# zxhuang1698/ZeroShape

Measured on AMD Instinct MI355X. Metric: sdf_query_points_per_sec_vox128, higher is better.
Workload: dtype f16x3

## Files before the change

### include/zeroshape_hip.h

```cpp
#ifndef ZEROSHAPE_HIP_H
#define ZEROSHAPE_HIP_H

#include <stddef.h>
#include <stdint.h>

#ifdef __cplusplus
extern "C" {
#endif

#define ZS_ABI_VERSION 41

int zs_abi_version(void);

const char *zs_last_error(void);


int zs_chamfer_forward(const float *xyz1, const float *xyz2, int b, int n, int m,
                       float *dist1, float *dist2, int *idx1, int *idx2, void *stream);

size_t zs_chamfer_workspace_bytes(int b, int n, int m);
int zs_chamfer_forward_ws(const float *xyz1, const float *xyz2, int b, int n, int m,
                          float *dist1, float *dist2, int *idx1, int *idx2,
                          void *workspace, size_t workspace_bytes, void *stream);

int zs_chamfer_backward(const float *xyz1, const float *xyz2, int b, int n, int m,
                        float *gradxyz1, float *gradxyz2,
                        const float *graddist1, const float *graddist2,
                        const int *idx1, const int *idx2, void *stream);


size_t zs_sdf_program_bytes(void);
size_t zs_sdf_prologue_scratch_bytes(void);
size_t zs_sdf_workspace_bytes(void);
size_t zs_sdf_attn_scratch_bytes(int batch, int m);

int zs_sdf_prologue(void *programs, size_t program_stride_bytes, const float *lat_params,
                    const float *latent_depth, int batch, void *scratch, void *stream);
#define ZS_SDF_POS_PERLAYER 1
int zs_sdf_prologue_ex(void *programs, size_t program_stride_bytes, const float *lat_params,
                       const float *latent_depth, int batch, void *scratch, int flags, void *stream);

int zs_sdf_verdict_stats(const float *got, const float *want, int batch, int m, float flip_band, float tol, float tol_occ,
                         float *stats, int *flags, void *stream);

int zs_sdf_query_points(const void *programs, size_t program_stride_bytes, int batch,
                        const float *points, int m, float *logits, float *attn,
                        const int *tile_mask, void *workspace, void *stream);

int zs_sdf_query_grid(const void *programs, size_t program_stride_bytes, int batch,
                      const float *axis, int G, int slice_begin, int slice_end,
                      int apply_sigmoid, float *out, const int *tile_mask, void *workspace,
                      void *stream);

size_t zs_sdf_grid_attn_zmean_scratch_bytes(int batch, int n_cols, int G, size_t cap_bytes);
int zs_sdf_grid_attn_zmean_chunk(int batch, int n_cols, int G, size_t cap_bytes, int *imgs_per_chunk ,
                                 int *cols_per_chunk );
int zs_sdf_grid_attn_zmean(const void *programs, size_t program_stride_bytes, int batch,
                           const float *axis, int G, const int *columns, int n_cols, float *zmean,
                           void *workspace, void *scratch, size_t scratch_bytes, void *stream);

int zs_attn_frames(const float *zmean, int batch, int n_cols, const int *frame_col, int n_frames,
                   const float *images, int H, int W, const uint8_t *lut, int R, float *frames, void *stream);

int zs_sdf_split_programs(const void *programs, size_t program_stride_bytes, void *split_programs,
                          size_t split_stride_bytes, int batch, void *stream);
int zs_sdf_query_points_split(const void *split_programs, size_t program_stride_bytes, int batch,
                              const float *points, int m, float *logits, int *tile_flags,
                              void *workspace, void *stream);
int zs_sdf_query_grid_split(const void *split_programs, size_t program_stride_bytes, int batch,
                            const float *axis, int G, int slice_begin, int slice_end,
                            int apply_sigmoid, float *out, int *tile_flags, void *workspace,
                            void *stream);

int zs_sdf_block0_tables(const void *split_programs, size_t program_stride_bytes, int batch, float *tables, void *stream);

int zs_sdf_query_grid_range(const void *programs, size_t program_stride_bytes, int batch,
                            const float *axis, int G, long long point_begin, long long point_end,
                            int apply_sigmoid, float *out, const int *tile_mask, void *workspace,
                            void *stream);
int zs_sdf_query_grid_range_split(const void *split_programs, size_t program_stride_bytes, int batch,
                                  const float *axis, int G, long long point_begin,
                                  long long point_end, int apply_sigmoid, float *out,
                                  int *tile_flags, void *workspace, void *stream);

size_t zs_bf_grid_bytes(void);
size_t zs_bf_scratch_bytes(void);
int zs_bf_lower_bounds(const float *pred, int n, const float *gt_normalized, int m,
                       const float *rotations, int k, float *grid_gt, float *grid_pred,
                       void *scratch, float *lower_bounds, void *stream);

int zs_pose_max_batch(void);
size_t zs_pose_scratch_bytes(int n, int m, int count);
size_t zs_pose_best_bytes(void);
int zs_pose_best_init(float *best, void *stream);
int zs_pose_search_batch(const float *pred, int n, const float *gt_normalized, int m,
                         const float *rotations, const int *order, int count, int index_offset,
                         const float *lower_bound, const float *thresholds6, float *best,
                         void *scratch, void *stream);
size_t zs_pose_grid_bytes(int n, int m, int count);
int zs_pose_gt_grid(const float *gt_normalized, int m, void *grids, void *stream);
int zs_pose_search_batch_grid(const float *pred, int n, const float *gt_normalized, int m, const float *rotations,
                              const int *order, int count, int index_offset, const float *lower_bound,
                              const float *thresholds6, float *best, void *scratch, void *grids, const float *pred_stats,
                              void *stream);
size_t zs_morton_scratch_bytes(int n);
int zs_morton_sort(const float *points, int n, float *sorted, int *perm, float *tile_boxes, int tile, void *scratch,
                   void *stream);
size_t zs_str_scratch_bytes(int n);
int zs_str_sort(const float *points, int n, float *sorted, int *perm, void *scratch, void *stream);
size_t zs_pose_pack_bytes(int points);
int zs_pose_pack(const float *sorted_points, int points, float *pack, void *stream);
size_t zs_pose_sorted_scratch_bytes(int n, int m, int count);
int zs_pose_search_batch_sorted(const float *pred, const float *pred_sorted, int n, const float *gt_sorted,
                                const float *gt_pack, int m, const float *rotations, const int *order, int count,
                                int index_offset, const float *lower_bound, const float *thresholds6, float *best,
                                void *scratch, int mode, void *stream);
int zs_pose_apply(const float *pred, int n, const float *rotations, const int *index, float *out,
                  void *scratch, void *stream);
int zs_normalize_pc(const float *pc, int b, int n, float *out, void *scratch, void *stream);
int zs_standardize_pc(const float *pc, int b, int n, float *out, void *stream);
size_t zs_icp_scratch_bytes(int b);
int zs_icp_step(const float *x1, int n, const float *x2, int m, const int *idx1, int b, float *x1_out, void *scratch,
                void *stream);
int zs_fscore(const float *dist1, int n, const float *dist2, int m, int b, const float *thresholds,
              int n_thresholds, float *out, void *stream);

size_t zs_mc_scratch_bytes(int G);
size_t zs_mesh_sample_scratch_doubles(int n_tris);
int zs_mc_count(const float *vol, int G, float iso, const uint8_t *tri_count, void *scratch,
                int *total, void *stream);
int zs_mc_emit(const float *vol, int G, float iso, const int8_t *tri_table, int table_stride,
               const uint8_t *tri_count, const void *scratch, float scale, float offset,
               float *tris, int n_tris, void *stream);
int zs_mesh_sample(const float *tris, int n_tris, int n_samples, uint64_t seed, double *cum_area,
                   float *points, void *stream);


size_t zs_mesh_stats_scratch_bytes(int n_tris);
int zs_mesh_stats(const float *tris, int n_tris, float *out, void *scratch, void *stream);

size_t zs_render_zbuffer_bytes(int frames, int H, int W);
int zs_render_frames(const float *tris, int n_tris, const float *xform, const float *cams,
                     int frames, int H, int W, float yfov, float znear, const float *base_rgb,
                     uint8_t *rgb, float *depth, int *tri, void *zbuffer, void *stream);

int zs_intr_param2mtx(const float *params, int batch, int H, int W, float *intr, void *stream);
int zs_unproj_depth(const float *depth, const float *intr, int batch, int H, int W, float *points,
                    void *stream);
int zs_valid_norm_fac(const float *points, const uint8_t *mask, int batch, int n, float *mean,
                      float *max_dist, void *stream);
int zs_masked_resample(const float *map, const float *mask, int batch, int channels, int H, int W,
                       int Ho, int Wo, float bg, float *out, float *mask_out, void *stream);
int zs_seen_surface(const float *depth, const float *intr, const float *mask, int batch, int H, int W,
                    int Ho, int Wo, float *seen_points, float *mean, float *scale, float *coord_dsp,
                    float *mask_dsp, void *stream);
size_t zs_seen_surface_workspace_bytes(int batch);
int zs_seen_surface_ws(const float *depth, const float *intr, const float *mask, int batch, int H, int W,
                       int Ho, int Wo, float *seen_points, float *mean, float *scale, float *coord_dsp,
                       float *mask_dsp, void *workspace, void *stream);

#define ZS_DEPTH_PRED_IS_DISPARITY 1
#define ZS_DEPTH_SOLVE_ONLY 2
int zs_depth_metrics(const float *prediction, const float *target, const float *mask, int batch, int n,
                     int flags, float depth_cap, const float *thresholds,
                     int n_thresholds, float *metrics, float *prediction_depth, float *scale_shift,
                     void *stream);

#define ZS_ACT_NONE 0
#define ZS_ACT_RELU 1
#define ZS_ACT_GELU 2
#define ZS_ACT_RELU_CLAMP1 3
#define ZS_ACT_SOFTPLUS 4
#define ZS_CONV_IN_RELU 1
#define ZS_CONV_FORCE_LARGE 2
#define ZS_CONV_FORCE_SMALL 4
#define ZS_CONV_F16X3 16
#define ZS_CONV_SPLIT_SMALL 32
#define ZS_CONV_STREAM_K 64
#define ZS_CONV_STREAM_K_ALWAYS 256
#define ZS_CONV_W_PRESPLIT 128
#define ZS_CONV_IN_DILATE2 8
#define ZS_CONV_FORCE_TILE256 1024
#define ZS_CONV_OUT_K16 2048
#define ZS_CONV_IN_K16 4096
#define ZS_CONV_IN_UPSAMPLE2 512
size_t zs_conv2d_packed_floats(int Cin, int Cout, int kh, int kw);
int zs_conv2d_presplit_weight(const float *packed_w, float *split_w, int Cin, int Cout, int kh, int kw, void *stream);
int zs_conv2d_presplit_weight_multi(const void *const *packed, void *const *split, const int *cout_pad,
                                    const unsigned long long *pair_prefix, int n, unsigned long long total_pairs,
                                    void *stream);
int zs_conv2d_nhwc(const float *in, const float *packed_w, const float *scale, const float *shift,
                   const float *res1, const float *res2, float *out, int batch, int Hin, int Win, int Cin,
                   int Hout, int Wout, int Cout, int kh, int kw, int stride, int pad_t, int pad_l, int flags,
                   float in_scale, float in_shift, int act, void *stream);
size_t zs_conv2d_splitk_workspace_bytes(void);
int zs_conv2d_nhwc_ws(const float *in, const float *packed_w, const float *scale, const float *shift,
                   const float *res1, const float *res2, float *out, int batch, int Hin, int Win, int Cin,
                   int Hout, int Wout, int Cout, int kh, int kw, int stride, int pad_t, int pad_l, int flags,
                   float in_scale, float in_shift, int act, void *workspace, void *stream);

typedef struct zs_conv_fuse {
    int in_mode, in_tiles, in_groups;
    int in_gshift;
    const float *in_stats, *in_gamma, *in_beta;
    float in_eps;
    int out_mode, out_groups;
    float *out_stats;
} zs_conv_fuse;
int zs_conv2d_nhwc_fused(const float *in, const float *packed_w, const float *scale, const float *shift,
                         const float *res1, const float *res2, float *out, int batch, int Hin, int Win,
                         int Cin, int Hout, int Wout, int Cout, int kh, int kw, int stride, int pad_t,
                         int pad_l, int flags, float in_scale, float in_shift, int act, const zs_conv_fuse *fuse,
                         void *workspace, void *stream);
int zs_conv2d_fused_cols(int M, int Cout);
int zs_conv2d_k16_ok(int M, int Cin, int Cout, int flags, int ln_in_tiles, int row_stats_out, int has_res);
int zs_gn_relu_max_pool_nhwc(const float *x, const float *stats, int tiles, const float *gamma, const float *beta,
                             float *table, float *y, int batch, int Hin, int Win, int C, int Hout, int Wout, int k,
                             int stride, int pad_t, int pad_l, float eps, void *stream);
int zs_group_norm_apply_stats(const float *x, const float *stats, int tiles, const float *gamma, const float *beta,
                              const float *residual, const float *res_stats, int res_tiles, const float *res_gamma,
                              const float *res_beta, float *y, int batch, int HW, int C, float eps, int relu, void *stream);
int zs_conv3x3_tail_nhwc(const float *in, const float *packed_w, const float *scale, const float *shift, float *out,
                         int batch, int H, int W, int Cin, int Cout, int flags, int act, const float *tail_w,
                         const float *tail_b, int tail_act, void *stream);
int zs_group_norm_nhwc(const float *x, const float *gamma, const float *beta, const float *residual, float *y,
                       int batch, int HW, int C, int groups, float eps, int relu, void *stream);
size_t zs_group_norm_workspace_bytes(int batch, int HW, int C, int groups);
int zs_group_norm_nhwc_ws(const float *x, const float *gamma, const float *beta, const float *residual, float *y,
                          int batch, int HW, int C, int groups, float eps, int relu, void *workspace, void *stream);
int zs_layer_norm(const float *x, const float *gamma, const float *beta, float *y, int rows, int C, float eps,
                  void *stream);
int zs_attention(const float *qkv, float *out, int batch, int L, int heads, int head_dim, void *stream);
int zs_attention_split(const float *qkv, float *out, int batch, int L, int heads, int head_dim, void *stream);
int zs_max_pool_nhwc(const float *x, float *y, int batch, int Hin, int Win, int C, int Hout, int Wout, int k,
                     int stride, int pad_t, int pad_l, void *stream);
int zs_global_mean_nhwc(const float *x, float *y, int batch, int HW, int C, void *stream);
int zs_upsample2x_nhwc(const float *x, float *y, int batch, int Hin, int Win, int C, void *stream);
int zs_nchw_to_nhwc(const float *x, const float *mask, float *y, int batch, int C, int HW, int Cpad,
                    void *stream);
int zs_nhwc_to_nchw(const float *x, float *y, int batch, int C, int HW, void *stream);
int zs_assemble_tokens(const float *feat, const float *cls, const float *pos, float *tokens, int batch, int n,
                       int C, void *stream);
int zs_readout_concat(const float *tokens, float *out, int batch, int n, int C, void *stream);
int zs_window_tokens(const float *emb, const uint8_t *mask, const float *invalid_token, const float *cls,
                     const float *pos, float *out, int batch, int H, int W, int C, int win, void *stream);

typedef struct zs_tensor_entry {
    float *param;
    const float *grad;
    float *exp_avg, *exp_avg_sq;
    unsigned long long n;
    float lr, weight_decay;
} zs_tensor_entry;

int zs_pack_conv_weight(const float *w, float *packed, int Cout, int Cin, int cin0, int CinTot, int kh, int kw,
                        int dgrad, void *stream);
typedef struct zs_pack_entry {
    const float *src;
    float *dst;
    int Cout, Cin, cin0, ld, taps, dgrad, K16, NPad;
} zs_pack_entry;
int zs_pack_chunk_elems(void);
int zs_pack_entry_chunks(int Cout, int Cin, int taps, int dgrad, int K16, int NPad);
int zs_pack_conv_weight_multi(const zs_pack_entry *table, const int *chunk_entry, const unsigned long long *chunk_start,
                              int n_chunks, void *stream);
int zs_pack_entry_inline_split(int Cout, int Cin, int taps, int dgrad);
int zs_pack_conv_weight_multi_split(const zs_pack_entry *table, const int *chunk_entry,
                                    const unsigned long long *chunk_start, int n_chunks, float *const *split_dst,
                                    int split_only, void *stream);
size_t zs_conv2d_wgrad_workspace_bytes(int batch, int Hout, int Wout, int Cin, int Cout, int kh, int kw);
int zs_conv2d_wgrad(const float *in, const float *dy, float *dw, float *db, void *workspace, int batch, int Hin, int Win,
                    int CinP, int Hout, int Wout, int Cout, int kh, int kw, int stride, int pad_t, int pad_l,
                    int flags, float in_scale, float in_shift, int Cin, int cin0, int CinTot, int accumulate,
                    void *stream);
int zs_conv2d_dgrad_small_cin(const float *dy, const float *w, float *dx, int batch, int H, int W, int CinP, int Hout,
                              int Wout, int Cout, int kh, int kw, int stride, int pad_t, int pad_l, int Cin, int cin0,
                              int CinTot, float scale, void *stream);
int zs_standardize_weight(const float *w, float *out, int Cout, int n, float eps, void *stream);
typedef struct zs_std_entry {
    const float *w;
    float *out;
    int rows, n;
    float eps;
    int pad;
} zs_std_entry;
int zs_standardize_weight_multi(const zs_std_entry *table, const int *row_prefix, int n_entries, int total_rows, void *stream);
int zs_standardize_weight_bwd(const float *w, const float *grad_out, float *dw, int Cout, int n, float eps,
                              void *stream);
int zs_act_forward(const float *x, float *y, size_t n, int act, float beta, void *stream);
int zs_act_backward(const float *dy, const float *ref, float *dx, size_t n, int act, float beta, void *stream);
int zs_posenc3d(const float *points, size_t n, int L, float *out, int stride, void *stream);
int zs_add_scaled_rows(const float *x, const float *branch, const float *scale, float *y, int batch,
                       size_t per_sample, void *stream);
size_t zs_column_sum_workspace_bytes(int rows, int C);
int zs_column_sum(const float *x, float *out, int rows, int C, float scale, void *workspace, void *stream);
size_t zs_layer_norm_bwd_workspace_bytes(int rows, int C);
int zs_layer_norm_bwd(const float *dy, const float *x, const float *gamma, float *dx, float *dgamma, float *dbeta,
                      int rows, int C, float eps, void *workspace, void *stream);
int zs_layer_norm_bwd_add(const float *dy, const float *x, const float *gamma, const float *add, float *dx, float *dgamma,
                          float *dbeta, int rows, int C, float eps, void *workspace, void *stream);
size_t zs_attention_bwd_workspace_bytes(int batch, int L, int heads);
int zs_attention_bwd(const float *qkv, const float *dout, float *dqkv, void *workspace, int batch, int L, int heads,
                     int head_dim, void *stream);
int zs_point_attention(const float *qkv_points, const float *qkv_latent, float *out, int batch, int M, int Ll,
                       int heads, int head_dim, void *stream);
int zs_point_attention_probs(const float *qkv_points, const float *qkv_latent, float *attn, int batch, int M, int Ll,
                             int heads, int head_dim, float weight, int accumulate, void *stream);
size_t zs_point_attention_bwd_workspace_bytes(int batch, int M, int Ll, int heads);
int zs_point_attention_bwd(const float *qkv_points, const float *qkv_latent, const float *dout, float *dqkv_points,
                           float *dqkv_latent, int accumulate_latent, void *workspace, int batch, int M, int Ll,
                           int heads, int head_dim, void *stream);
size_t zs_bce_logits_workspace_bytes(size_t n);
int zs_bce_logits(const float *logits, const float *sdf, size_t n, float impt_thres, float impt_weight, float *loss,
                  void *workspace, void *stream);
int zs_bce_logits_bwd(const float *logits, const float *sdf, size_t n, float impt_thres, float impt_weight,
                      const float *grad_loss, float *dlogits, void *stream);
int zs_erode_mask(const float *mask, int batch, int H, int W, int pool, float *out, void *stream);
size_t zs_midas_loss_workspace_bytes(int batch);
int zs_midas_loss(const float *prediction, const float *target, const float *mask, int batch, int H, int W, float alpha,
                  int scales, int inverse_depth, float *loss, void *workspace, void *stream);
int zs_midas_loss_bwd(const float *prediction, const float *target, const float *mask, int batch, int H, int W,
                      float alpha, int scales, int inverse_depth, const void *workspace, const float *grad_loss,
                      float *dprediction, void *stream);
int zs_intr_loss(const float *seen_pred, const float *seen_gt, const float *mask, size_t n, float *out2, void *stream);
int zs_intr_loss_bwd(const float *seen_pred, const float *seen_gt, const float *mask, size_t n, const float *out2,
                     const float *grad_loss, float *dseen_pred, void *stream);
int zs_multi_tensor_chunk_elems(void);
int zs_adamw_multi(const zs_tensor_entry *table, const int *chunk_tensor, const unsigned long long *chunk_start,
                   int n_chunks, float beta1, float beta2, float eps, int step, const float *grad_scale,
                   const int *skipped_steps, void *stream);
int zs_copy_multi(const zs_tensor_entry *table, const int *chunk_tensor, const unsigned long long *chunk_start,
                  int n_chunks, float scale, void *stream);
int zs_sumsq_multi(const zs_tensor_entry *table, const int *chunk_tensor, const unsigned long long *chunk_start,
                   int n_chunks, float *partial, float *sumsq, void *stream);

size_t zs_batch_norm_workspace_bytes(int rows, int C);
int zs_batch_norm_train(const float *x, const float *gamma, const float *beta, const float *residual, float *y,
                        float *running_mean, float *running_var, float *save_mean, float *save_rstd, int rows, int C,
                        float eps, float momentum, int relu, void *workspace, void *stream);
int zs_batch_norm_bwd(const float *x, const float *dy, const float *y_relu, const float *gamma, const float *save_mean,
                      const float *save_rstd, float *dx, float *dresidual, float *dgamma, float *dbeta, int rows, int C,
                      void *workspace, void *stream);
size_t zs_group_norm_bwd_workspace_bytes(int batch, int C);
int zs_group_norm_bwd(const float *x, const float *dy, const float *y_relu, const float *gamma, float *dx,
                      float *dresidual, float *dgamma, float *dbeta, int batch, int HW, int C, int groups, float eps,
                      void *workspace, void *stream);
int zs_max_pool_bwd_nhwc(const float *x, const float *dy, float *dx, int batch, int Hin, int Win, int C, int Hout,
                         int Wout, int k, int stride, int pad_t, int pad_l, void *stream);
int zs_global_mean_bwd_nhwc(const float *dy, float *dx, int batch, int HW, int C, void *stream);
int zs_upsample2x_bwd_nhwc(const float *dy, float *dx, int batch, int Hin, int Win, int C, void *stream);
int zs_nhwc_to_nchw_masked(const float *x, const float *mask, float *y, int batch, int C, int HW, int Cpad,
                           void *stream);
int zs_seen_surface_bwd(const float *depth, const float *intr, const float *mask, const float *mean, const float *scale,
                        const float *d_seen_points, const float *d_coord_dsp, int batch, int H, int W, float *d_depth,
                        float *d_intr, void *stream);
int zs_intr_param2mtx_bwd(const float *params, const float *d_intr, int batch, int H, int W, float *d_params,
                          void *stream);
int zs_window_tokens_bwd(const float *d_out, const uint8_t *mask, float *d_emb, float *d_inv_rows, float *d_cls_rows,
                         int batch, int H, int W, int C, int win, void *stream);
int zs_coord_dsp2_bwd(const float *d_dsp, const float *mask, const float *mask_dsp, float *d_full, int batch, int H,
                      int W, void *stream);
int zs_transform_points(const float *points, const float *pose, const float *mean, const float *scale, float *out,
                        int batch, int n, void *stream);
int zs_resize_bilinear_nhwc(const float *x, float *y, int Hi, int Wi, int Ho, int Wo, int C, int backward,
                            void *stream);
int zs_readout_concat_bwd(const float *dout, float *dtokens, int batch, int n, int C, void *stream);

#ifdef __cplusplus
}
#endif
#endif
```

### zeroshape_amd/_lib.py

```python
import contextlib
import ctypes
import os

_HERE = os.path.dirname(os.path.abspath(__file__))
LIB_PATH = os.environ.get("ZS_LIB_PATH") or os.path.join(_HERE, "libzeroshape_hip.so")

_c_void_p = ctypes.c_void_p
_c_int = ctypes.c_int
_c_size_t = ctypes.c_size_t
_c_float = ctypes.c_float

class ConvFuse(ctypes.Structure):
    _fields_ = [("in_mode", ctypes.c_int), ("in_tiles", ctypes.c_int), ("in_groups", ctypes.c_int), ("in_gshift", ctypes.c_int),
                ("in_stats", ctypes.c_void_p), ("in_gamma", ctypes.c_void_p), ("in_beta", ctypes.c_void_p),
                ("in_eps", ctypes.c_float), ("out_mode", ctypes.c_int), ("out_groups", ctypes.c_int),
                ("out_stats", ctypes.c_void_p)]


SIGNATURES = {
    "zs_abi_version": (_c_int, []),
    "zs_last_error": (ctypes.c_char_p, []),
    "zs_chamfer_forward": (_c_int, [_c_void_p, _c_void_p, _c_int, _c_int, _c_int,
                                    _c_void_p, _c_void_p, _c_void_p, _c_void_p, _c_void_p]),
    "zs_chamfer_workspace_bytes": (_c_size_t, [_c_int, _c_int, _c_int]),
    "zs_chamfer_forward_ws": (_c_int, [_c_void_p, _c_void_p, _c_int, _c_int, _c_int,
                                       _c_void_p, _c_void_p, _c_void_p, _c_void_p, _c_void_p, _c_size_t,
                                       _c_void_p]),
    "zs_chamfer_backward": (_c_int, [_c_void_p, _c_void_p, _c_int, _c_int, _c_int,
                                     _c_void_p, _c_void_p, _c_void_p, _c_void_p,
                                     _c_void_p, _c_void_p, _c_void_p]),
    "zs_sdf_program_bytes": (_c_size_t, []),
    "zs_sdf_prologue_scratch_bytes": (_c_size_t, []),
    "zs_sdf_workspace_bytes": (_c_size_t, []),
    "zs_sdf_attn_scratch_bytes": (_c_size_t, [_c_int, _c_int]),
    "zs_sdf_prologue": (_c_int, [_c_void_p, _c_size_t, _c_void_p, _c_void_p, _c_int,
                                 _c_void_p, _c_void_p]),
    "zs_sdf_prologue_ex": (_c_int, [_c_void_p, _c_size_t, _c_void_p, _c_void_p, _c_int,
                                    _c_void_p, _c_int, _c_void_p]),
    "zs_sdf_verdict_stats": (_c_int, [_c_void_p, _c_void_p, _c_int, _c_int, _c_float, _c_float, _c_float, _c_void_p, _c_void_p,
                                      _c_void_p]),
    "zs_sdf_query_points": (_c_int, [_c_void_p, _c_size_t, _c_int, _c_void_p, _c_int,
                                     _c_void_p, _c_void_p, _c_void_p, _c_void_p, _c_void_p]),
    "zs_sdf_query_grid": (_c_int, [_c_void_p, _c_size_t, _c_int, _c_void_p, _c_int, _c_int,
                                   _c_int, _c_int, _c_void_p, _c_void_p, _c_void_p, _c_void_p]),
    "zs_sdf_grid_attn_zmean_scratch_bytes": (_c_size_t, [_c_int, _c_int, _c_int, _c_size_t]),
    "zs_sdf_grid_attn_zmean_chunk": (_c_int, [_c_int, _c_int, _c_int, _c_size_t, ctypes.POINTER(_c_int),
                                              ctypes.POINTER(_c_int)]),
    "zs_sdf_grid_attn_zmean": (_c_int, [_c_void_p, _c_size_t, _c_int, _c_void_p, _c_int, _c_void_p, _c_int, _c_void_p,
                                        _c_void_p, _c_void_p, _c_size_t, _c_void_p]),
    "zs_attn_frames": (_c_int, [_c_void_p, _c_int, _c_int, _c_void_p, _c_int, _c_void_p, _c_int, _c_int, _c_void_p, _c_int,
                                _c_void_p, _c_void_p]),
    "zs_sdf_split_programs": (_c_int, [_c_void_p, _c_size_t, _c_void_p, _c_size_t, _c_int, _c_void_p]),
    "zs_sdf_block0_tables": (_c_int, [_c_void_p, _c_size_t, _c_int, _c_void_p, _c_void_p]),
    "zs_sdf_query_points_split": (_c_int, [_c_void_p, _c_size_t, _c_int, _c_void_p, _c_int,
                                           _c_void_p, _c_void_p, _c_void_p, _c_void_p]),
    "zs_sdf_query_grid_split": (_c_int, [_c_void_p, _c_size_t, _c_int, _c_void_p, _c_int, _c_int,
                                         _c_int, _c_int, _c_void_p, _c_void_p, _c_void_p, _c_void_p]),
    "zs_sdf_query_grid_range": (_c_int, [_c_void_p, _c_size_t, _c_int, _c_void_p, _c_int, ctypes.c_longlong,
                                         ctypes.c_longlong, _c_int, _c_void_p, _c_void_p, _c_void_p, _c_void_p]),
    "zs_sdf_query_grid_range_split": (_c_int, [_c_void_p, _c_size_t, _c_int, _c_void_p, _c_int,
                                               ctypes.c_longlong, ctypes.c_longlong, _c_int, _c_void_p,
                                               _c_void_p, _c_void_p, _c_void_p]),
    "zs_erode_mask": (_c_int, [_c_void_p, _c_int, _c_int, _c_int, _c_int, _c_void_p, _c_void_p]),
    "zs_bf_grid_bytes": (_c_size_t, []),
    "zs_bf_scratch_bytes": (_c_size_t, []),
    "zs_bf_lower_bounds": (_c_int, [_c_void_p, _c_int, _c_void_p, _c_int, _c_void_p, _c_int, _c_void_p,
                                    _c_void_p, _c_void_p, _c_void_p, _c_void_p]),
    "zs_pose_max_batch": (_c_int, []),
    "zs_pose_scratch_bytes": (_c_size_t, [_c_int, _c_int, _c_int]),
    "zs_pose_best_bytes": (_c_size_t, []),
    "zs_pose_best_init": (_c_int, [_c_void_p, _c_void_p]),
    "zs_pose_search_batch": (_c_int, [_c_void_p, _c_int, _c_void_p, _c_int, _c_void_p, _c_void_p, _c_int, _c_int,
                                      _c_void_p, _c_void_p, _c_void_p, _c_void_p, _c_void_p]),
    "zs_pose_grid_bytes": (_c_size_t, [_c_int, _c_int, _c_int]),
    "zs_pose_gt_grid": (_c_int, [_c_void_p, _c_int, _c_void_p, _c_void_p]),
    "zs_pose_search_batch_grid": (_c_int, [_c_void_p, _c_int, _c_void_p, _c_int, _c_void_p, _c_void_p, _c_int, _c_int,
                                           _c_void_p, _c_void_p, _c_void_p, _c_void_p, _c_void_p, _c_void_p, _c_void_p]),
    "zs_morton_scratch_bytes": (_c_size_t, [_c_int]),
    "zs_morton_sort": (_c_int, [_c_void_p, _c_int, _c_void_p, _c_void_p, _c_void_p, _c_int, _c_void_p, _c_void_p]),
    "zs_str_scratch_bytes": (_c_size_t, [_c_int]),
    "zs_str_sort": (_c_int, [_c_void_p, _c_int, _c_void_p, _c_void_p, _c_void_p, _c_void_p]),
    "zs_pose_pack_bytes": (_c_size_t, [_c_int]),
    "zs_pose_pack": (_c_int, [_c_void_p, _c_int, _c_void_p, _c_void_p]),
    "zs_pose_sorted_scratch_bytes": (_c_size_t, [_c_int, _c_int, _c_int]),
    "zs_pose_search_batch_sorted": (_c_int, [_c_void_p, _c_void_p, _c_int, _c_void_p, _c_void_p, _c_int, _c_void_p,
                                             _c_void_p, _c_int, _c_int, _c_void_p, _c_void_p, _c_void_p, _c_void_p,
                                             _c_int, _c_void_p]),
    "zs_pose_apply": (_c_int, [_c_void_p, _c_int, _c_void_p, _c_void_p, _c_void_p, _c_void_p, _c_void_p]),
    "zs_standardize_pc": (_c_int, [_c_void_p, _c_int, _c_int, _c_void_p, _c_void_p]),
    "zs_icp_scratch_bytes": (_c_size_t, [_c_int]),
    "zs_icp_step": (_c_int, [_c_void_p, _c_int, _c_void_p, _c_int, _c_void_p, _c_int, _c_void_p, _c_void_p, _c_void_p]),
    "zs_normalize_pc": (_c_int, [_c_void_p, _c_int, _c_int, _c_void_p, _c_void_p, _c_void_p]),
    "zs_fscore": (_c_int, [_c_void_p, _c_int, _c_void_p, _c_int, _c_int, _c_void_p, _c_int, _c_void_p, _c_void_p]),
    "zs_mc_scratch_bytes": (_c_size_t, [_c_int]),
    "zs_mesh_sample_scratch_doubles": (_c_size_t, [_c_int]),
    "zs_mc_count": (_c_int, [_c_void_p, _c_int, ctypes.c_float, _c_void_p, _c_void_p, _c_void_p, _c_void_p]),
    "zs_mc_emit": (_c_int, [_c_void_p, _c_int, ctypes.c_float, _c_void_p, _c_int, _c_void_p, _c_void_p,
                            ctypes.c_float, ctypes.c_float, _c_void_p, _c_int, _c_void_p]),
    "zs_mesh_sample": (_c_int, [_c_void_p, _c_int, _c_int, ctypes.c_uint64, _c_void_p, _c_void_p, _c_void_p]),
    "zs_mesh_stats_scratch_bytes": (_c_size_t, [_c_int]),
    "zs_mesh_stats": (_c_int, [_c_void_p, _c_int, _c_void_p, _c_void_p, _c_void_p]),
    "zs_render_zbuffer_bytes": (_c_size_t, [_c_int, _c_int, _c_int]),
    "zs_render_frames": (_c_int, [_c_void_p, _c_int, ctypes.POINTER(_c_float), _c_void_p, _c_int, _c_int, _c_int, _c_float,
                                  _c_float, ctypes.POINTER(_c_float), _c_void_p, _c_void_p, _c_void_p, _c_void_p, _c_void_p]),
    "zs_intr_param2mtx": (_c_int, [_c_void_p, _c_int, _c_int, _c_int, _c_void_p, _c_void_p]),
    "zs_unproj_depth": (_c_int, [_c_void_p, _c_void_p, _c_int, _c_int, _c_int, _c_void_p, _c_void_p]),
    "zs_valid_norm_fac": (_c_int, [_c_void_p, _c_void_p, _c_int, _c_int, _c_void_p, _c_void_p, _c_void_p]),
    "zs_masked_resample": (_c_int, [_c_void_p, _c_void_p, _c_int, _c_int, _c_int, _c_int, _c_int, _c_int,
                                    ctypes.c_float, _c_void_p, _c_void_p, _c_void_p]),
    "zs_seen_surface": (_c_int, [_c_void_p, _c_void_p, _c_void_p, _c_int, _c_int, _c_int, _c_int, _c_int,
                                 _c_void_p, _c_void_p, _c_void_p, _c_void_p, _c_void_p, _c_void_p]),
    "zs_seen_surface_workspace_bytes": (_c_size_t, [_c_int]),
    "zs_seen_surface_ws": (_c_int, [_c_void_p, _c_void_p, _c_void_p, _c_int, _c_int, _c_int, _c_int, _c_int,
                                    _c_void_p, _c_void_p, _c_void_p, _c_void_p, _c_void_p, _c_void_p, _c_void_p]),
    "zs_depth_metrics": (_c_int, [_c_void_p, _c_void_p, _c_void_p, _c_int, _c_int, _c_int, ctypes.c_float,
                                  ctypes.POINTER(ctypes.c_float), _c_int, _c_void_p, _c_void_p, _c_void_p,
                                  _c_void_p]),
    "zs_conv2d_packed_floats": (_c_size_t, [_c_int, _c_int, _c_int, _c_int]),
    "zs_conv2d_presplit_weight": (_c_int, [_c_void_p, _c_void_p, _c_int, _c_int, _c_int, _c_int, _c_void_p]),
    "zs_conv2d_nhwc": (_c_int, [_c_void_p] * 7 + [_c_int] * 13 + [ctypes.c_float, ctypes.c_float, _c_int,
                                                                  _c_void_p]),
    "zs_conv2d_splitk_workspace_bytes": (_c_size_t, []),
    "zs_conv2d_presplit_weight_multi": (_c_int, [_c_void_p] * 4 + [_c_int, ctypes.c_ulonglong, _c_void_p]),
    "zs_conv3x3_tail_nhwc": (_c_int, [_c_void_p] * 5 + [_c_int] * 7 + [_c_void_p, _c_void_p, _c_int, _c_void_p]),
    "zs_conv2d_nhwc_ws": (_c_int, [_c_void_p] * 7 + [_c_int] * 13 + [ctypes.c_float, ctypes.c_float, _c_int,
                                                                     _c_void_p, _c_void_p]),
    "zs_conv2d_nhwc_fused": (_c_int, [_c_void_p] * 7 + [_c_int] * 13 + [ctypes.c_float, ctypes.c_float, _c_int,
                                                                        _c_void_p, _c_void_p, _c_void_p]),
    "zs_conv2d_fused_cols": (_c_int, [_c_int, _c_int]),
    "zs_conv2d_k16_ok": (_c_int, [_c_int] * 7),
    "zs_gn_relu_max_pool_nhwc": (_c_int, [_c_void_p, _c_void_p, _c_int] + [_c_void_p] * 4 + [_c_int] * 10 + [ctypes.c_float, _c_void_p]),
    "zs_group_norm_apply_stats": (_c_int, [_c_void_p, _c_void_p, _c_int] + [_c_void_p] * 4 + [_c_int] + [_c_void_p] * 3 +
                                  [_c_int, _c_int, _c_int, ctypes.c_float, _c_int, _c_void_p]),
    "zs_group_norm_nhwc": (_c_int, [_c_void_p] * 5 + [_c_int, _c_int, _c_int, _c_int, ctypes.c_float, _c_int,
                                                      _c_void_p]),
    "zs_group_norm_workspace_bytes": (_c_size_t, [_c_int, _c_int, _c_int, _c_int]),
    "zs_group_norm_nhwc_ws": (_c_int, [_c_void_p] * 5 + [_c_int, _c_int, _c_int, _c_int, ctypes.c_float, _c_int,
                                       _c_void_p, _c_void_p]),
    "zs_layer_norm": (_c_int, [_c_void_p] * 4 + [_c_int, _c_int, ctypes.c_float, _c_void_p]),
    "zs_attention": (_c_int, [_c_void_p, _c_void_p, _c_int, _c_int, _c_int, _c_int, _c_void_p]),
    "zs_attention_split": (_c_int, [_c_void_p, _c_void_p, _c_int, _c_int, _c_int, _c_int, _c_void_p]),
    "zs_max_pool_nhwc": (_c_int, [_c_void_p, _c_void_p] + [_c_int] * 10 + [_c_void_p]),
    "zs_global_mean_nhwc": (_c_int, [_c_void_p, _c_void_p, _c_int, _c_int, _c_int, _c_void_p]),
    "zs_upsample2x_nhwc": (_c_int, [_c_void_p, _c_void_p, _c_int, _c_int, _c_int, _c_int, _c_void_p]),
    "zs_nchw_to_nhwc": (_c_int, [_c_void_p, _c_void_p, _c_void_p, _c_int, _c_int, _c_int, _c_int, _c_void_p]),
    "zs_window_tokens": (_c_int, [_c_void_p] * 6 + [_c_int] * 5 + [_c_void_p]),
    "zs_nhwc_to_nchw": (_c_int, [_c_void_p, _c_void_p, _c_int, _c_int, _c_int, _c_void_p]),
    "zs_assemble_tokens": (_c_int, [_c_void_p] * 4 + [_c_int, _c_int, _c_int, _c_void_p]),
    "zs_readout_concat": (_c_int, [_c_void_p, _c_void_p, _c_int, _c_int, _c_int, _c_void_p]),
    "zs_pack_conv_weight": (_c_int, [_c_void_p, _c_void_p] + [_c_int] * 7 + [_c_void_p]),
    "zs_pack_chunk_elems": (_c_int, []),
    "zs_pack_entry_chunks": (_c_int, [_c_int] * 6),
    "zs_pack_conv_weight_multi": (_c_int, [_c_void_p, _c_void_p, _c_void_p, _c_int, _c_void_p]),
    "zs_pack_entry_inline_split": (_c_int, [_c_int] * 4),
    "zs_pack_conv_weight_multi_split": (_c_int, [_c_void_p, _c_void_p, _c_void_p, _c_int, _c_void_p, _c_int, _c_void_p]),
    "zs_conv2d_wgrad_workspace_bytes": (_c_size_t, [_c_int] * 7),
    "zs_conv2d_wgrad": (_c_int, [_c_void_p] * 5 + [_c_int] * 13 + [_c_float, _c_float] + [_c_int] * 4 + [_c_void_p]),
    "zs_conv2d_dgrad_small_cin": (_c_int, [_c_void_p] * 3 + [_c_int] * 15 + [_c_float, _c_void_p]),
    "zs_standardize_weight": (_c_int, [_c_void_p, _c_void_p, _c_int, _c_int, _c_float, _c_void_p]),
    "zs_standardize_weight_multi": (_c_int, [_c_void_p, _c_void_p, _c_int, _c_int, _c_void_p]),
    "zs_standardize_weight_bwd": (_c_int, [_c_void_p, _c_void_p, _c_void_p, _c_int, _c_int, _c_float, _c_void_p]),
    "zs_act_forward": (_c_int, [_c_void_p, _c_void_p, _c_size_t, _c_int, _c_float, _c_void_p]),
    "zs_act_backward": (_c_int, [_c_void_p, _c_void_p, _c_void_p, _c_size_t, _c_int, _c_float, _c_void_p]),
    "zs_posenc3d": (_c_int, [_c_void_p, _c_size_t, _c_int, _c_void_p, _c_int, _c_void_p]),
    "zs_add_scaled_rows": (_c_int, [_c_void_p] * 4 + [_c_int, _c_size_t, _c_void_p]),
    "zs_column_sum_workspace_bytes": (_c_size_t, [_c_int, _c_int]),
    "zs_column_sum": (_c_int, [_c_void_p, _c_void_p, _c_int, _c_int, _c_float, _c_void_p, _c_void_p]),
    "zs_layer_norm_bwd_workspace_bytes": (_c_size_t, [_c_int, _c_int]),
    "zs_layer_norm_bwd": (_c_int, [_c_void_p] * 6 + [_c_int, _c_int, _c_float, _c_void_p, _c_void_p]),
    "zs_layer_norm_bwd_add": (_c_int, [_c_void_p] * 7 + [_c_int, _c_int, _c_float, _c_void_p, _c_void_p]),
    "zs_attention_bwd_workspace_bytes": (_c_size_t, [_c_int, _c_int, _c_int]),
    "zs_attention_bwd": (_c_int, [_c_void_p] * 4 + [_c_int] * 4 + [_c_void_p]),
    "zs_point_attention": (_c_int, [_c_void_p] * 3 + [_c_int] * 5 + [_c_void_p]),
    "zs_point_attention_probs": (_c_int, [_c_void_p, _c_void_p, _c_void_p, _c_int, _c_int, _c_int, _c_int, _c_int, _c_float, _c_int,
                                          _c_void_p]),
    "zs_point_attention_bwd_workspace_bytes": (_c_size_t, [_c_int] * 4),
    "zs_point_attention_bwd": (_c_int, [_c_void_p] * 5 + [_c_int, _c_void_p] + [_c_int] * 5 + [_c_void_p]),
    "zs_bce_logits_workspace_bytes": (_c_size_t, [_c_size_t]),
    "zs_bce_logits": (_c_int, [_c_void_p, _c_void_p, _c_size_t, _c_float, _c_float, _c_void_p, _c_void_p,
                               _c_void_p]),
    "zs_bce_logits_bwd": (_c_int, [_c_void_p, _c_void_p, _c_size_t, _c_float, _c_float, _c_void_p, _c_void_p,
                                   _c_void_p]),
    "zs_midas_loss_workspace_bytes": (_c_size_t, [_c_int]),
    "zs_midas_loss": (_c_int, [_c_void_p] * 3 + [_c_int] * 3 + [_c_float, _c_int, _c_int, _c_void_p, _c_void_p, _c_void_p]),
    "zs_midas_loss_bwd": (_c_int, [_c_void_p] * 3 + [_c_int] * 3 + [_c_float, _c_int, _c_int, _c_void_p, _c_void_p,
                                                                    _c_void_p, _c_void_p]),
    "zs_intr_loss": (_c_int, [_c_void_p] * 3 + [_c_size_t, _c_void_p, _c_void_p]),
    "zs_intr_loss_bwd": (_c_int, [_c_void_p] * 3 + [_c_size_t] + [_c_void_p] * 4),
    "zs_multi_tensor_chunk_elems": (_c_int, []),
    "zs_adamw_multi": (_c_int, [_c_void_p, _c_void_p, _c_void_p, _c_int, _c_float, _c_float, _c_float, _c_int,
                                _c_void_p, _c_void_p, _c_void_p]),
    "zs_copy_multi": (_c_int, [_c_void_p, _c_void_p, _c_void_p, _c_int, _c_float, _c_void_p]),
    "zs_sumsq_multi": (_c_int, [_c_void_p, _c_void_p, _c_void_p, _c_int, _c_void_p, _c_void_p, _c_void_p]),
    "zs_batch_norm_workspace_bytes": (_c_size_t, [_c_int, _c_int]),
    "zs_batch_norm_train": (_c_int, [_c_void_p] * 9 + [_c_int, _c_int, _c_float, _c_float, _c_int, _c_void_p,
                                                       _c_void_p]),
    "zs_batch_norm_bwd": (_c_int, [_c_void_p] * 10 + [_c_int, _c_int, _c_void_p, _c_void_p]),
    "zs_group_norm_bwd_workspace_bytes": (_c_size_t, [_c_int, _c_int]),
    "zs_group_norm_bwd": (_c_int, [_c_void_p] * 8 + [_c_int, _c_int, _c_int, _c_int, _c_float, _c_void_p, _c_void_p]),
    "zs_max_pool_bwd_nhwc": (_c_int, [_c_void_p] * 3 + [_c_int] * 10 + [_c_void_p]),
    "zs_global_mean_bwd_nhwc": (_c_int, [_c_void_p, _c_void_p, _c_int, _c_int, _c_int, _c_void_p]),
    "zs_upsample2x_bwd_nhwc": (_c_int, [_c_void_p, _c_void_p, _c_int, _c_int, _c_int, _c_int, _c_void_p]),
    "zs_nhwc_to_nchw_masked": (_c_int, [_c_void_p, _c_void_p, _c_void_p, _c_int, _c_int, _c_int, _c_int, _c_void_p]),
    "zs_seen_surface_bwd": (_c_int, [_c_void_p] * 7 + [_c_int, _c_int, _c_int, _c_void_p, _c_void_p, _c_void_p]),
    "zs_intr_param2mtx_bwd": (_c_int, [_c_void_p, _c_void_p, _c_int, _c_int, _c_int, _c_void_p, _c_void_p]),
    "zs_window_tokens_bwd": (_c_int, [_c_void_p] * 5 + [_c_int] * 5 + [_c_void_p]),
    "zs_coord_dsp2_bwd": (_c_int, [_c_void_p] * 4 + [_c_int] * 3 + [_c_void_p]),
    "zs_transform_points": (_c_int, [_c_void_p] * 5 + [_c_int, _c_int, _c_void_p]),
    "zs_resize_bilinear_nhwc": (_c_int, [_c_void_p, _c_void_p] + [_c_int] * 6 + [_c_void_p]),
    "zs_readout_concat_bwd": (_c_int, [_c_void_p, _c_void_p, _c_int, _c_int, _c_int, _c_void_p]),
}

ABI_VERSION = 41
_lib = None


class ZeroShapeHipError(RuntimeError):
    pass


def load():
    global _lib
    if _lib is not None:
        return _lib
    if not os.path.exists(LIB_PATH):
        raise ZeroShapeHipError(
            "HIP library not built: %s is missing (run `python -m zeroshape_amd.build`). "
            "zeroshape_amd has no CPU/PyTorch fallback for this path." % LIB_PATH)
    import torch
    try:
        lib = ctypes.CDLL(LIB_PATH)
    except OSError as e:
        raise ZeroShapeHipError("cannot load %s: %s" % (LIB_PATH, e)) from e
    for name, (res, args) in SIGNATURES.items():
        try:
            fn = getattr(lib, name)
        except AttributeError as e:
            raise ZeroShapeHipError("%s does not export %s" % (LIB_PATH, name)) from e
        fn.restype = res
        fn.argtypes = args
    v = lib.zs_abi_version()
    if v != ABI_VERSION:
        raise ZeroShapeHipError("ABI mismatch: library %d, binding %d" % (v, ABI_VERSION))
    _lib = lib
    return lib


CALLS = [0]


def check(rc, what):
    CALLS[0] += 1
    if rc != 1:
        msg = load().zs_last_error()
        raise ZeroShapeHipError("%s failed: %s" % (what, (msg or b"").decode(errors="replace")))


def ptr(t):
    return None if t is None else ctypes.c_void_p(t.data_ptr())


def current_stream_ptr(device=None):
    import torch
    idx = getattr(device, "index", device)
    if idx is None:
        idx = torch.cuda.current_device()
    return ctypes.c_void_p(torch._C._cuda_getCurrentRawStream(idx))


_NULL_GUARD = contextlib.nullcontext()


def on(device):
    import torch
    idx = getattr(device, "index", device)
    if idx is None or idx == torch.cuda.current_device():
        return _NULL_GUARD
    return torch.cuda.device(device)
```

### zeroshape_amd/csrc/sdf_decoder_split.hip

```cpp
#include "zs_common.h"
#include <stdlib.h>
#include "sdf_layout.h"
#include "sdf_math.h"
#include "zs_split16.h"
#include "../../include/zeroshape_hip.h"

#include <math.h>
#include <stdint.h>
#include <type_traits>

namespace {

using namespace zs::lay;
using zs::dm::gelu_erf;
using zs::dm::softplus100;

typedef float f32x16 __attribute__((ext_vector_type(16)));
typedef float f32x4 __attribute__((ext_vector_type(4)));
typedef float f32x2 __attribute__((ext_vector_type(2)));
typedef unsigned u32x4 __attribute__((ext_vector_type(4)));

constexpr float S_GUARD = 64.0f;
constexpr int WAVES = 4;
constexpr int PTS_PER_WAVE = 32;
constexpr int PTS_PER_BLOCK = WAVES * PTS_PER_WAVE;
constexpr int MAX_WGS = 256;
constexpr int KB_U4 = 128;
constexpr int CK = 8;
constexpr int KPW = CK / WAVES;
constexpr int CHUNK_BYTES = CK * KB_U4 * 16;
constexpr int NBUF = 2;
constexpr int KB_TOTAL = G_TOTAL / 2;
constexpr int PRM_WINDOW = 4096;
constexpr int STAGE_FLOATS = NBUF * CHUNK_BYTES / 4;
constexpr int SLAB_TILES = NT - 1;
constexpr int SLAB_U4 = SLAB_TILES * 4 * 64;
constexpr int ZTILES_F4 = NT * 4 * 64;
constexpr int ZSLAB_F4 = 3 * ZTILES_F4;
constexpr int LDS_FLOATS = PRM_WINDOW + STAGE_FLOATS + WAVES * SLAB_U4 * 4;
static_assert(LDS_FLOATS * 4 == 160 * 1024, "the kernel owns the whole LDS of a CU");
static_assert(KB_TOTAL % CK == 0 && CK % WAVES == 0 && KPW * 2048 <= 4096, "chunking");
static_assert((RING * GROUP_FLOATS + PARAM_FLOATS) * 4 >= NBUF * CHUNK_BYTES, "prefetch stays inside the program");

constexpr int W_PP = P_PP;
constexpr int W_BLK = P_BLK0;
constexpr int W_IA = P_LNFG;
constexpr int W_IB = P_IMPL_PAIR + P_IMPL_PAIR_STRIDE;
static_assert(P_BLK_STRIDE <= PRM_WINDOW && W_IB - W_IA <= PRM_WINDOW && P_USED - W_IB <= PRM_WINDOW,
              "params windows");

#define DEV __device__ __forceinline__
#ifdef ZS_FENCE_SCHED
#define ZS_FENCE __builtin_amdgcn_sched_barrier(0)
#else
#define ZS_FENCE do { } while (0)
#endif

DEV void pin(u32x4 &a, u32x4 &b) { asm volatile("" : "+v"(a), "+v"(b) : : "memory"); }

using zs::s16::mfma3;
using zs::s16::split2;

struct PT {
    u32x4 v[4];
};
template <typename T>
DEV PT pack_tile(const T &x) {
    PT p;
#pragma unroll
    for (int j = 0; j < 2; j++)
#pragma unroll
        for (int i = 0; i < 4; i++) {
            unsigned h, l;
            split2(x[8 * j + 2 * i], x[8 * j + 2 * i + 1], h, l);
            p.v[2 * j][i] = h;
            p.v[2 * j + 1][i] = l;
        }
    return p;
}

DEV void glds_kblocks(const char *gsrc, unsigned lds_dst) {
#ifdef ZS_EXP_NO_DMA
    if (gsrc != nullptr) return;
#endif
#ifndef ZS_DMA_MOD
#define ZS_DMA_MOD ""
#endif
    asm volatile("s_mov_b32 m0, %1\n\ts_nop 0\n\tglobal_load_lds_dwordx4 %0, off" ZS_DMA_MOD
                 "\n\tglobal_load_lds_dwordx4 %0, off offset:1024" ZS_DMA_MOD
                 "\n\tglobal_load_lds_dwordx4 %0, off offset:2048" ZS_DMA_MOD
                 "\n\tglobal_load_lds_dwordx4 %0, off offset:3072" ZS_DMA_MOD
                 :
                 : "v"(gsrc), "s"(lds_dst)
                 : "memory");
}

struct AStream {
    const u32x4 *buf[NBUF];
    unsigned dst[NBUF];
    u32x4 hi, lo;
    const char *gsrc;

    DEV void init(const char *prog, u32x4 *stage, unsigned stage_addr, int wave, int lane, int first_byte = 0) {
        const char *g = prog + first_byte + wave * (KPW * KB_U4 * 16) + lane * 16;
        asm volatile("s_waitcnt vmcnt(0) lgkmcnt(0)\n\ts_barrier" ::: "memory");
#pragma unroll
        for (int i = 0; i < NBUF; i++) {
            buf[i] = stage + i * (CK * KB_U4) + lane;
            dst[i] = stage_addr + i * CHUNK_BYTES + wave * (KPW * KB_U4 * 16);
            glds_kblocks(g + i * CHUNK_BYTES, dst[i]);
        }
        gsrc = g + NBUF * CHUNK_BYTES;
        asm volatile("s_waitcnt vmcnt(4)\n\ts_barrier" ::: "memory");
        hi = buf[0][0];
        lo = buf[0][64];
    }
    template <int EXTRA_VM = 0>
    DEV void step(int pos, u32x4 &ahi, u32x4 &alo) {
        ahi = hi;
        alo = lo;
        if (pos == CK - 1) {
            static_assert(EXTRA_VM == 0 || EXTRA_VM == 4, "wait-count variants");
            if (EXTRA_VM == 4)
                asm volatile("s_waitcnt vmcnt(4) lgkmcnt(0)\n\ts_barrier" ::: "memory");
            else
                asm volatile("s_waitcnt vmcnt(0) lgkmcnt(0)\n\ts_barrier" ::: "memory");
            glds_kblocks(gsrc, dst[0]);
            gsrc += CHUNK_BYTES;
            const u32x4 *t = buf[0];
            const unsigned u = dst[0];
            buf[0] = buf[1];
            dst[0] = dst[1];
            buf[1] = t;
            dst[1] = u;
            hi = buf[0][0];
            lo = buf[0][64];
        } else {
#ifndef ZS_EXP_NO_AREAD
            hi = buf[0][(pos + 1) * KB_U4];
            lo = buf[0][(pos + 1) * KB_U4 + 64];
#endif
        }
    }
    DEV void skip(int bytes) { gsrc += bytes; }
    DEV void drain() { asm volatile("s_waitcnt vmcnt(0) lgkmcnt(0)" ::: "memory"); }
};

struct Slab {
    u32x4 *fl;
    PT t7;
    DEV void store(int tile, const PT &p) {
        if (tile == SLAB_TILES) {
            t7 = p;
        } else {
#pragma unroll
            for (int q = 0; q < 4; q++) fl[(tile * 4 + q) * 64] = p.v[q];
        }
    }
};

DEV f32x16 zero16() {
    f32x16 v;
#pragma unroll
    for (int r = 0; r < 16; r++) v[r] = 0.f;
    return v;
}

struct NoSide {
    DEV void operator()(int, int) const {}
};
template <typename SIDE>
DEV void mfma3_gaps(f32x16 &acc, const u32x4 &ahi, const u32x4 &alo, const u32x4 &bhi, const u32x4 &blo, int kb,
                    SIDE &side) {
    using zs::s16::as_h;
    if (std::is_same<SIDE, NoSide>::value) {
        mfma3(acc, ahi, alo, bhi, blo);
        return;
    }
    acc = __builtin_amdgcn_mfma_f32_32x32x16_f16(as_h(alo), as_h(bhi), acc, 0, 0, 0);
    ZS_FENCE;
    side(kb, 0);
    ZS_FENCE;
    acc = __builtin_amdgcn_mfma_f32_32x32x16_f16(as_h(ahi), as_h(blo), acc, 0, 0, 0);
    ZS_FENCE;
    side(kb, 1);
    ZS_FENCE;
    acc = __builtin_amdgcn_mfma_f32_32x32x16_f16(as_h(ahi), as_h(bhi), acc, 0, 0, 0);
    ZS_FENCE;
    side(kb, 2);
    ZS_FENCE;
}

struct TilePacker {
    PT p;
    float prev;
    DEV void feed(int kb, float v) {
        if (kb & 1) {
            unsigned h, l;
            split2(prev, v, h, l);
            p.v[2 * (kb >> 3)][(kb & 7) >> 1] = h;
            p.v[2 * (kb >> 3) + 1][(kb & 7) >> 1] = l;
        }
        prev = v;
    }
};

struct GeluStager {
    float x, u, q, t, e, p;
    DEV void s0(float v) {
        x = v;
        u = fabsf(v) * 0.70710678118654752440f;
        q = (u * u) * -1.44269504088896340736f;
    }
    DEV void s1() { t = __builtin_amdgcn_rcpf(fmaf(0.3275911f, u, 1.0f)); }
    DEV void s2() {
        e = __builtin_amdgcn_exp2f(q);
        p = fmaf(0.75052702f, t, -1.02753365f);
    }
    DEV void s3() {
        p = fmaf(p, t, 1.00509130f);
        p = fmaf(p, t, -0.20116957f);
        p = fmaf(p, t, 0.18019173f);
        p = p * t;
        u = u * p;
    }
    DEV float s4() const { return fmaf(-u, e, fmaxf(x, 0.0f)); }
    DEV float all(float v) {
        s0(v); s1(); s2(); s3();
        return s4();
    }
    DEV void stage(int st, float v, int idx, TilePacker &pk) {
        if (st == 0) s0(v);
        else if (st == 1) s1();
        else if (st == 2) s2();
        else if (st == 3) s3();
        else if (st == 4) pk.feed(idx, s4());
    }
};
struct SoftplusStager {
    float x, t;
    DEV void s0(float v) {
        x = v;
        t = __builtin_amdgcn_exp2f(fabsf(v) * -144.26950408889634074f);
    }
    DEV void s1() { t = __builtin_amdgcn_logf(1.0f + t); }
    DEV float s2() const { return fmaf(t, 0.0069314718055994530942f, fmaxf(x, 0.0f)); }
};

DEV float kblock_gelu(f32x16 &acc, const u32x4 &ahi, const u32x4 &alo, const u32x4 &bhi, const u32x4 &blo, float x) {
    float u, q, d, t, e, m, p;
    const float c0 = 0.70710678118654752440f, c1 = 0.3275911f, c2 = -1.02753365f;
    asm volatile(
#ifndef ZS_EXP_TWO_TERM
                 "v_mfma_f32_32x32x16_f16 %[acc], %[alo], %[bh], %[acc]\n\t"
#endif
                 "v_mul_f32_e64 %[u], |%[x]|, %[c0]\n\t"
                 "v_mul_f32_e32 %[q], %[u], %[u]\n\t"
                 "v_mul_f32_e32 %[q], 0xbfb8aa3b, %[q]\n\t"
                 "v_fma_f32 %[d], %[u], %[c1], 1.0\n\t"
                 "v_mfma_f32_32x32x16_f16 %[acc], %[ahi], %[bl], %[acc]\n\t"
                 "v_rcp_f32_e32 %[t], %[d]\n\t"
                 "v_exp_f32_e32 %[e], %[q]\n\t"
                 "v_max_f32_e32 %[m], 0, %[x]\n\t"
                 "v_mfma_f32_32x32x16_f16 %[acc], %[ahi], %[bh], %[acc]\n\t"
                 "v_fmamk_f32 %[p], %[t], 0x3f40228a, %[c2]\n\t"
                 "v_fmaak_f32 %[p], %[p], %[t], 0x3f80a6d5\n\t"
                 "v_fmaak_f32 %[p], %[p], %[t], 0xbe4dff65\n\t"
                 "v_fmaak_f32 %[p], %[p], %[t], 0x3e38842e\n\t"
                 "v_mul_f32_e64 %[p], %[t], -%[p]\n\t"
                 "v_mul_f32_e32 %[p], %[u], %[p]\n\t"
                 "v_fmac_f32_e32 %[m], %[p], %[e]"
                 : [acc] "+v"(acc), [u] "=&v"(u), [q] "=&v"(q), [d] "=&v"(d), [t] "=&v"(t), [e] "=&v"(e), [m] "=&v"(m),
                   [p] "=&v"(p)
                 : [alo] "v"(alo), [ahi] "v"(ahi), [bh] "v"(bhi), [bl] "v"(blo), [x] "v"(x), [c0] "s"(c0), [c1] "s"(c1),
                   [c2] "v"(c2));
    return m;
}
DEV float kblock_softplus(f32x16 &acc, const u32x4 &ahi, const u32x4 &alo, const u32x4 &bhi, const u32x4 &blo, float x) {
    float t, m;
    const float c0 = -144.26950408889634074f;
    asm volatile(
#ifndef ZS_EXP_TWO_TERM
                 "v_mfma_f32_32x32x16_f16 %[acc], %[alo], %[bh], %[acc]\n\t"
#endif
                 "v_mul_f32_e64 %[t], |%[x]|, %[c0]\n\t"
                 "v_exp_f32_e32 %[t], %[t]\n\t"
                 "v_mfma_f32_32x32x16_f16 %[acc], %[ahi], %[bl], %[acc]\n\t"
                 "v_max_f32_e32 %[m], 0, %[x]\n\t"
                 "v_add_f32_e32 %[t], 1.0, %[t]\n\t"
                 "v_log_f32_e32 %[t], %[t]\n\t"
                 "v_mfma_f32_32x32x16_f16 %[acc], %[ahi], %[bh], %[acc]\n\t"
                 "s_nop 0\n\t"
                 "v_fmac_f32_e32 %[m], 0x3be32166, %[t]"
                 : [acc] "+v"(acc), [t] "=&v"(t), [m] "=&v"(m)
                 : [alo] "v"(alo), [ahi] "v"(ahi), [bh] "v"(bhi), [bl] "v"(blo), [x] "v"(x), [c0] "s"(c0));
    return m;
}

DEV void mfma_settle(f32x16 &acc) { asm volatile("s_nop 7\n\ts_nop 3" : "+v"(acc)); }

template <int KT, int EXTRA_VM = 0, typename SIDE = NoSide>
DEV void gemm_reg(AStream &s, const PT *X, f32x16 &acc, SIDE side = SIDE()) {
#pragma unroll
    for (int kt = 0; kt < KT; kt++)
#pragma unroll
        for (int j = 0; j < 2; j++) {
            u32x4 ahi, alo;
            s.step((kt * 2 + j) & (CK - 1), ahi, alo);
            pin(ahi, alo);
            mfma3_gaps(acc, ahi, alo, X[kt].v[2 * j], X[kt].v[2 * j + 1], kt * 2 + j, side);
        }
}
template <typename SIDE>
DEV void mfma3_breg(f32x16 &acc, const u32x4 &ahi, const u32x4 &alo, const u32x4 &bhi, const u32x4 &blo, int kb,
                    SIDE &side) {
    asm volatile("s_nop 1\n\tv_mfma_f32_32x32x16_f16 %0, %1, %2, %0" : "+v"(acc) : "v"(alo), "a"(bhi));
    ZS_FENCE;
    side(kb, 0);
    ZS_FENCE;
    asm volatile("s_nop 1\n\tv_mfma_f32_32x32x16_f16 %0, %1, %2, %0" : "+v"(acc) : "v"(ahi), "a"(blo));
    ZS_FENCE;
    side(kb, 1);
    ZS_FENCE;
    asm volatile("s_nop 1\n\tv_mfma_f32_32x32x16_f16 %0, %1, %2, %0" : "+v"(acc) : "v"(ahi), "a"(bhi));
    ZS_FENCE;
    side(kb, 2);
    ZS_FENCE;
}
template <int KT, typename SIDE = NoSide>
DEV void gemm_areg(AStream &s, const PT *X, f32x16 &acc, SIDE side = SIDE()) {
#pragma unroll
    for (int kt = 0; kt < KT; kt++)
#pragma unroll
        for (int j = 0; j < 2; j++) {
            u32x4 ahi, alo;
            s.step((kt * 2 + j) & (CK - 1), ahi, alo);
            pin(ahi, alo);
            mfma3_breg(acc, ahi, alo, X[kt].v[2 * j], X[kt].v[2 * j + 1], kt * 2 + j, side);
        }
}
template <typename SIDE>
DEV void mfma3_cacc(f32x16 &acc, const u32x4 &ahi, const u32x4 &alo, const u32x4 &bhi, const u32x4 &blo, int kb,
                    SIDE &side) {
    asm volatile("s_nop 1\n\tv_mfma_f32_32x32x16_f16 %0, %1, %2, %0" : "+a"(acc) : "v"(alo), "v"(bhi));
    ZS_FENCE;
    side(kb, 0);
    ZS_FENCE;
    asm volatile("s_nop 1\n\tv_mfma_f32_32x32x16_f16 %0, %1, %2, %0" : "+a"(acc) : "v"(ahi), "v"(blo));
    ZS_FENCE;
    side(kb, 1);
    ZS_FENCE;
    asm volatile("s_nop 1\n\tv_mfma_f32_32x32x16_f16 %0, %1, %2, %0" : "+a"(acc) : "v"(ahi), "v"(bhi));
    ZS_FENCE;
    side(kb, 2);
    ZS_FENCE;
}
template <bool YACC = false, typename SIDE = NoSide>
DEV void gemm_one(AStream &s, const PT &X, f32x16 &acc, int pos0, int kb0 = 0, SIDE side = SIDE()) {
#pragma unroll
    for (int j = 0; j < 2; j++) {
        u32x4 ahi, alo;
        s.step((pos0 + j) & (CK - 1), ahi, alo);
        pin(ahi, alo);
        if (YACC)
            mfma3_cacc(acc, ahi, alo, X.v[2 * j], X.v[2 * j + 1], kb0 + j, side);
        else
            mfma3_gaps(acc, ahi, alo, X.v[2 * j], X.v[2 * j + 1], kb0 + j, side);
    }
}
DEV void slab_b(const Slab &sl, int kb, u32x4 &bh, u32x4 &bl) {
    if (kb >= SLAB_TILES * 2) {
        bh = sl.t7.v[(kb & 1) * 2];
        bl = sl.t7.v[(kb & 1) * 2 + 1];
    } else {
        bh = sl.fl[kb * KB_U4];
        bl = sl.fl[kb * KB_U4 + 64];
    }
}
template <typename SIDE = NoSide>
DEV void gemm_lds(AStream &s, const Slab &sl, f32x16 &acc, int pos0 = 0, SIDE side = SIDE()) {
    u32x4 bh, bl;
    slab_b(sl, 0, bh, bl);
#pragma unroll
    for (int kb = 0; kb < NT * 2; kb++) {
        u32x4 ahi, alo;
        s.step((pos0 + kb) & (CK - 1), ahi, alo);
        u32x4 nh = bh, nl = bl;
        if (kb + 1 < NT * 2) slab_b(sl, kb + 1, nh, nl);
        pin(ahi, alo);
        mfma3_gaps(acc, ahi, alo, bh, bl, kb, side);
        bh = nh;
        bl = nl;
    }
}

template <int ACT, typename FIN, typename TAIL>
DEV void gemm_lds_act(AStream &s, const Slab &sl, f32x16 &acc, const f32x16 &cur, FIN fin, TAIL tail) {
    u32x4 bh, bl;
    slab_b(sl, 0, bh, bl);
#pragma unroll
    for (int kb = 0; kb < NT * 2; kb++) {
        u32x4 ahi, alo;
        s.step(kb & (CK - 1), ahi, alo);
        u32x4 nh = bh, nl = bl;
        if (kb + 1 < NT * 2) slab_b(sl, kb + 1, nh, nl);
        const float r = ACT == 0 ? kblock_gelu(acc, ahi, alo, bh, bl, cur[kb]) : kblock_softplus(acc, ahi, alo, bh, bl, cur[kb]);
        bh = nh;
        bl = nl;
        fin(kb, r);
        tail(kb);
    }
}
template <int ACT, typename FIN, typename TAIL>
DEV void gemm_reg_act(AStream &s, const PT *X, f32x16 &acc, const f32x16 &cur, FIN fin, TAIL tail) {
#pragma unroll
    for (int kt = 0; kt < NT; kt++)
#pragma unroll
        for (int j = 0; j < 2; j++) {
            u32x4 ahi, alo;
            const int kb = kt * 2 + j;
            s.step(kb & (CK - 1), ahi, alo);
            const float r = ACT == 0 ? kblock_gelu(acc, ahi, alo, X[kt].v[2 * j], X[kt].v[2 * j + 1], cur[kb])
                                     : kblock_softplus(acc, ahi, alo, X[kt].v[2 * j], X[kt].v[2 * j + 1], cur[kb]);
            fin(kb, r);
            tail(kb);
        }
}

#ifndef ZS_SPLIT_PERMLANE
DEV float half_sum(float v) { return v + __shfl_xor(v, 32, 64); }
DEV float half_max(float v) { return fmaxf(v, __shfl_xor(v, 32, 64)); }
#else
DEV void half_pair(float v, float &lo, float &hi) {
    lo = v;
    hi = v;
    asm volatile("s_nop 4\n\tv_permlane32_swap_b32 %0, %1\n\ts_nop 4" : "+v"(lo), "+v"(hi));
}
DEV float half_sum(float v) {
    float lo, hi;
    half_pair(v, lo, hi);
    return lo + hi;
}
#ifdef ZS_SPLIT_PERMLANE_SUM_ONLY
DEV float half_max(float v) { return fmaxf(v, __shfl_xor(v, 32, 64)); }
#else
DEV float half_max(float v) {
    float lo, hi;
    half_pair(v, lo, hi);
    return fmaxf(lo, hi);
}
#endif
#endif

DEV void rp(const float *prm, int off, int tile, int hi, float *v) {
    const f32x4 *q = reinterpret_cast<const f32x4 *>(prm + off + tile * 32 + hi * 16);
#pragma unroll
    for (int i = 0; i < 4; i++) {
        const f32x4 a = q[i];
        v[4 * i + 0] = a.x; v[4 * i + 1] = a.y; v[4 * i + 2] = a.z; v[4 * i + 3] = a.w;
    }
}
DEV f32x16 rp16(const float *prm, int off, int tile, int hi) {
    float t[16];
    rp(prm, off, tile, hi, t);
    f32x16 v;
#pragma unroll
    for (int r = 0; r < 16; r++) v[r] = t[r];
    return v;
}
constexpr int B0_BPROJ = 0, B0_C = 256, B0_T = 1024;
static_assert(B0_T + HEADS * 3 * 128 == PRM_WINDOW, "the block-0 table is exactly one params window");
DEV f32x16 block0_qkv(const float *prm, int tile, int hi, float xr, float yr, float zr, float rstd) {
    f32x16 v = rp16(prm, B0_C, tile, hi);
    const f32x4 *q = reinterpret_cast<const f32x4 *>(prm + B0_T + tile * 128 + hi * 64);
#pragma unroll
    for (int r = 0; r < 16; r++) {
        const f32x4 w = q[r];
        v[r] = fmaf(w.z, zr, fmaf(w.y, yr, fmaf(w.x, xr, fmaf(w.w, rstd, v[r]))));
    }
    return v;
}
DEV f32x16 xyz_affine(const float *prm, int off, int tile, int hi, float x, float y, float z) {
    const f32x4 *q = reinterpret_cast<const f32x4 *>(prm + off + tile * 128 + hi * 64);
    f32x16 v;
#pragma unroll
    for (int r = 0; r < 16; r++) {
        const f32x4 w = q[r];
        v[r] = fmaf(w.z, z, fmaf(w.y, y, fmaf(w.x, x, w.w)));
    }
    return v;
}

struct XyzInit {
    const f32x4 *q;
    f32x4 w;
    f32x16 v;
    DEV void start(const float *prm, int off, int tile, int hi) {
        q = reinterpret_cast<const f32x4 *>(prm + off + tile * 128 + hi * 64);
        w = q[0];
    }
    DEV void step(int r, float x, float y, float z) {
        v[r] = fmaf(w.z, z, fmaf(w.y, y, fmaf(w.x, x, w.w)));
        if (r + 1 < 16) w = q[r + 1];
    }
};
struct RowInit {
    const f32x4 *q;
    f32x4 w;
    f32x16 v;
    DEV void start(const float *prm, int off, int tile, int hi) {
        q = reinterpret_cast<const f32x4 *>(prm + off + tile * 32 + hi * 16);
        w = q[0];
    }
    DEV void step(int r) {
        if ((r & 3) == 0) {
            v[r] = w.x; v[r + 1] = w.y; v[r + 2] = w.z; v[r + 3] = w.w;
            if (r + 4 < 16) w = q[(r >> 2) + 1];
        }
    }
};

DEV void ln_stats(const f32x16 *x, float &mean, float &rstd) {
    float s = 0.f;
#pragma unroll
    for (int kt = 0; kt < NT; kt++)
#pragma unroll
        for (int r = 0; r < 16; r++) s += x[kt][r];
    s = half_sum(s);
    mean = s * (1.0f / 256.0f);
    float v = 0.f;
#pragma unroll
    for (int kt = 0; kt < NT; kt++)
#pragma unroll
        for (int r = 0; r < 16; r++) {
            const float d = x[kt][r] - mean;
            v = fmaf(d, d, v);
        }
    v = half_sum(v);
    rstd = 1.0f / sqrtf(v * (1.0f / 256.0f) + 1e-6f);
}
DEV void layer_norm_lds(const f32x16 *x, Slab &sl, const float *prm, int g_off, int b_off, int hi) {
    float mean, rstd;
    ln_stats(x, mean, rstd);
#pragma unroll
    for (int kt = 0; kt < NT; kt++) {
        float g[16], b[16], t[16];
        rp(prm, g_off, kt, hi, g);
        rp(prm, b_off, kt, hi, b);
#pragma unroll
        for (int r = 0; r < 16; r++) t[r] = fmaf((x[kt][r] - mean) * rstd, g[r], b[r]);
        sl.store(kt, pack_tile(t));
    }
}

DEV void load_params(float *prm, const float *prog_params, int start, int count) {
    __syncthreads();
    const f32x4 *src = reinterpret_cast<const f32x4 *>(prog_params + start);
    f32x4 *dst = reinterpret_cast<f32x4 *>(prm);
    for (int i = threadIdx.x; i < count / 4; i += WAVES * 64) dst[i] = src[i];
    __syncthreads();
}

template <bool MASK>
DEV void attn_tile(AStream &s, const PT &q, f32x16 &o, float &m_run, float &z_run, float c, int hi,
                   int pos0) {
    f32x16 S = zero16();
    gemm_one(s, q, S, pos0);
    float mt = -INFINITY;
#pragma unroll
    for (int r = 0; r < 16; r++) {
        if (MASK) {
            const int rw = (r & 3) + 8 * (r >> 2) + 4 * hi;
            S[r] = rw < L - 32 * (LT - 1) ? S[r] : -INFINITY;
        }
        mt = fmaxf(mt, S[r]);
    }
    mt *= c;
    constexpr float LAZY = 8.0f;
    if (__builtin_amdgcn_ballot_w64(mt > m_run + LAZY) != 0) {
        mt = half_max(mt);
        const float m_new = fmaxf(m_run, mt);
        const float alpha = __builtin_amdgcn_exp2f(m_run - m_new);
        z_run *= alpha;
#pragma unroll
        for (int r = 0; r < 16; r++) o[r] *= alpha;
        m_run = m_new;
    }
    float zs_ = 0.f;
#pragma unroll
    for (int r = 0; r < 16; r++) {
        const float p = __builtin_amdgcn_exp2f(fmaf(S[r], c, -m_run));
        S[r] = p;
        zs_ += p;
    }
    z_run += zs_;
    gemm_one(s, pack_tile(S), o, pos0 + 2);
}

#ifdef ZS_EXP_TIMING
#define ZS_STAMP(i) do { if (dbg) dbg[i] = __builtin_amdgcn_s_memtime(); } while (0)
#else
#define ZS_STAMP(i) do { } while (0)
#endif
DEV float decode_tile(const char *prog, float *prm, u32x4 *stage, unsigned stage_addr, u32x4 *slab,
                      const float *tbl, float px, float py, float pz, int wave, int lane, float &guard,
                      unsigned long long *dbg) {
    const int hi = lane >> 5;
    const float *prog_params = reinterpret_cast<const float *>(prog) + REC_FLOATS;
    constexpr int QKV_BYTES = 3 * NT * 2 / CK * CHUNK_BYTES;
    static_assert(3 * NT * 2 % CK == 0, "AStream::skip passes whole chunks");
    AStream s;
    s.init(prog, stage, stage_addr, wave, lane, tbl ? QKV_BYTES : 0);
    Slab sl;
    sl.fl = slab;
    ZS_STAMP(0);

    load_params(prm, prog_params, W_PP, 1024);
    f32x16 y[NT];
#pragma unroll
    for (int kt = 0; kt < NT; kt++) y[kt] = xyz_affine(prm, 0, kt, hi, px, py, pz);

    ZS_STAMP(1);

    const float scale = 0.17677669529663688110f;

#pragma unroll 1
    for (int blk = 0; blk < BLOCKS; blk++) {
        const bool tab = blk == 0 && tbl != nullptr;
        float rstd0 = 0.f, xr = 0.f, yr = 0.f, zr = 0.f;
        if (tab) {
            load_params(prm, tbl, 0, PRM_WINDOW);
            float mean;
            ln_stats(y, mean, rstd0);
            xr = px * rstd0;
            yr = py * rstd0;
            zr = pz * rstd0;
        } else {
            load_params(prm, prog_params, W_BLK + blk * P_BLK_STRIDE, P_BLK_STRIDE);
            layer_norm_lds(y, sl, prm, PB_LN1G, PB_LN1B, hi);
        }
        ZS_STAMP(2 + blk * 4);
#pragma unroll
        for (int nt = 0; nt < NT; nt++) y[nt] += rp16(prm, tab ? B0_BPROJ : PB_BPROJ, nt, hi);

        auto head = [&](int hd, auto Ptag) {
            constexpr int P = decltype(Ptag)::value;
            f32x16 q, k, v;
            if (tab) {
                q = block0_qkv(prm, hd * 3 + 0, hi, xr, yr, zr, rstd0);
                k = block0_qkv(prm, hd * 3 + 1, hi, xr, yr, zr, rstd0);
                v = block0_qkv(prm, hd * 3 + 2, hi, xr, yr, zr, rstd0);
            } else {
                q = rp16(prm, PB_BQKV, hd * 3 + 0, hi);
                gemm_lds(s, sl, q, P);
                k = rp16(prm, PB_BQKV, hd * 3 + 1, hi);
                gemm_lds(s, sl, k, P);
                v = rp16(prm, PB_BQKV, hd * 3 + 2, hi);
                gemm_lds(s, sl, v, P);
            }

            const float c = scale * 1.44269504088896340736f;
            float s_self = 0.f;
            float qq = 0.f;
#pragma unroll
            for (int r = 0; r < 16; r++) {
                s_self = fmaf(q[r], k[r], s_self);
                qq = fmaf(q[r], q[r], qq);
            }
            s_self = half_sum(s_self) * c;
            {
                const float km = prog_params[P_KMAX + blk * HEADS + hd] * scale;
                guard = fmaxf(guard, half_sum(qq) * (km * km));
            }
            const PT qp = pack_tile(q);

            float m_run = -INFINITY, z_run = 0.f;
            f32x16 o = zero16();
#pragma unroll 1
            for (int l2 = 0; l2 < (LT - 1) / 2; l2++) {
                attn_tile<false>(s, qp, o, m_run, z_run, c, hi, P);
                attn_tile<false>(s, qp, o, m_run, z_run, c, hi, (P + 4) & (CK - 1));
            }
            attn_tile<true>(s, qp, o, m_run, z_run, c, hi, P);
            {
                const float m_new = fmaxf(m_run, s_self);
                const float alpha = __builtin_amdgcn_exp2f(m_run - m_new);
                const float p_self = __builtin_amdgcn_exp2f(s_self - m_new);
                const float z = fmaf(half_sum(z_run), alpha, p_self);
                const float inv = 1.0f / z;
                const float a_i = alpha * inv, p_i = p_self * inv;
#pragma unroll
                for (int r = 0; r < 16; r++) o[r] = fmaf(p_i, v[r], o[r] * a_i);
            }
            const PT op = pack_tile(o);
            const bool bump = tab && hd + 1 < HEADS;
            if (bump && (P == 4 || wave >= 2)) s.skip(QKV_BYTES);
#pragma unroll
            for (int nt = 0; nt < NT; nt++) {
                if (P == 0 && nt == 2 && bump && wave < 2) s.skip(QKV_BYTES);
                gemm_one(s, op, y[nt], (P + 4 + 2 * nt) & (CK - 1));
            }
        };
        static_assert((LT - 1) % 2 == 0 && (3 * NT * 2 + LT * 4 + NT * 2) % CK == 4, "head = 11.5 chunks");
#pragma unroll 1
        for (int hd = 0; hd < HEADS; hd += 2) {
            head(hd, std::integral_constant<int, 0>());
            head(hd + 1, std::integral_constant<int, 4>());
        }

        ZS_STAMP(3 + blk * 4);
        if (tab) load_params(prm, prog_params, W_BLK, P_BLK_STRIDE);
        layer_norm_lds(y, sl, prm, PB_LN2G, PB_LN2B, hi);
#pragma unroll
        for (int nt = 0; nt < NT; nt++) y[nt] += rp16(prm, PB_B2, nt, hi);
        ZS_STAMP(4 + blk * 4);
        RowInit bi;
        f32x16 hid = rp16(prm, PB_B1, 0, hi);
        bi.start(prm, PB_B1, 1, hi);
        gemm_lds(s, sl, hid, 0, [&](int kb, int g) {
            if (g == 2 && (kb & 3) == 1) bi.step(kb & ~3);
        });
#pragma unroll 1
        for (int ht = 0; ht < HT - 1; ht++) {
            f32x16 nxt = bi.v;
            bi.start(prm, PB_B1, ht + 2 < HT ? ht + 2 : HT - 1, hi);
            TilePacker e;
            gemm_lds_act<0>(s, sl, nxt, hid, [&](int kb, float r) { e.feed(kb, r); },
                            [&](int kb) { if ((kb & 3) == 1) bi.step(kb & ~3); });
#pragma unroll
            for (int nt = 0; nt < NT; nt++) gemm_one(s, e.p, y[nt], (2 * nt) & (CK - 1));
            hid = nxt;
        }
        {
#pragma unroll
            for (int r = 0; r < 16; r++) hid[r] = gelu_erf(hid[r]);
            const PT hp = pack_tile(hid);
#pragma unroll
            for (int nt = 0; nt < NT; nt++) gemm_one(s, hp, y[nt], (2 * nt) & (CK - 1));
        }
        ZS_STAMP(5 + blk * 4);
    }

    load_params(prm, prog_params, W_IA, W_IB - W_IA);
    float h[NT * 16];
    {
        float mean, rstd;
        ln_stats(y, mean, rstd);
#pragma unroll
        for (int kt = 0; kt < NT; kt++) {
            float g[16], b[16];
            rp(prm, P_LNFG - W_IA, kt, hi, g);
            rp(prm, P_LNFB - W_IA, kt, hi, b);
#pragma unroll
            for (int r = 0; r < 16; r++) h[kt * 16 + r] = fmaf((y[kt][r] - mean) * rstd, g[r], b[r]);
        }
    }
    ZS_STAMP(10);
    PT hp[NT];

#pragma unroll
    for (int kt = 0; kt < NT; kt++) hp[kt] = pack_tile(h + kt * 16);
    {
        f32x16 prev;
        XyzInit ini;
        ini.v = xyz_affine(prm, P_IMPL0 - W_IA, 0, hi, px, py, pz);
#pragma unroll
        for (int nt = 0; nt <= NT; nt++) {
            TilePacker e;
            if (nt < NT) {
                f32x16 acc = ini.v;
                if (nt + 1 < NT) ini.start(prm, P_IMPL0 - W_IA, nt + 1, hi);
                if (nt > 0)
                    gemm_reg_act<1>(s, hp, acc, prev, [&](int kb, float r) { e.feed(kb, r); },
                                    [&](int kb) { if (nt + 1 < NT) ini.step(kb, px, py, pz); });
                else
                    gemm_reg<NT, 0>(s, hp, acc, [&](int kb, int g) { if (g == 2) ini.step(kb, px, py, pz); });
                if (nt > 0) sl.store(nt - 1, e.p);
                prev = acc;
            } else {
                mfma_settle(prev);
#pragma unroll
                for (int kb = 0; kb < 16; kb++) e.feed(kb, softplus100(prev[kb]));
                sl.store(nt - 1, e.p);
            }
        }
    }
    ZS_STAMP(11);
    const float rsqrt2 = 0.70710678118654752440f;
    PT fp[NT];
#pragma unroll
    for (int kt = 0; kt < NT; kt++) {
        float t[16];
#pragma unroll
        for (int r = 0; r < 16; r++) t[r] = h[kt * 16 + r] * rsqrt2;
        fp[kt] = pack_tile(t);
    }
    const float sx = px * rsqrt2, sy = py * rsqrt2, sz = pz * rsqrt2;

    ZS_STAMP(12);
    {
        f32x16 prev;
        RowInit ini;
        ini.v = rp16(prm, P_IMPL1 - W_IA, 0, hi);
#pragma unroll
        for (int nt = 0; nt <= NT; nt++) {
            TilePacker e;
            if (nt < NT) {
                f32x16 acc = ini.v;
                if (nt + 1 < NT) ini.start(prm, P_IMPL1 - W_IA, nt + 1, hi);
                if (nt > 0)
                    gemm_lds_act<1>(s, sl, acc, prev, [&](int kb, float r) { e.feed(kb, r * rsqrt2); },
                                    [&](int kb) { if (nt + 1 < NT) ini.step(kb); });
                else
                    gemm_lds(s, sl, acc, 0, [&](int kb, int g) { if (g == 2) ini.step(kb); });
                if (nt > 0) hp[nt - 1] = e.p;
                prev = acc;
            } else {
                mfma_settle(prev);
#pragma unroll
                for (int kb = 0; kb < 16; kb++) e.feed(kb, softplus100(prev[kb]) * rsqrt2);
                hp[nt - 1] = e.p;
            }
        }
    }
    ZS_STAMP(13);
    float out = 0.f;
#pragma unroll 1
    for (int i = 0; i < 3; i++) {
        if (i == 1) load_params(prm, prog_params, W_IB, P_USED - W_IB);
        const int pp = i == 0 ? P_IMPL_PAIR - W_IA : (i - 1) * P_IMPL_PAIR_STRIDE;
        {
            f32x16 prev;
            XyzInit ini;
            ini.v = xyz_affine(prm, pp, 0, hi, sx, sy, sz);
#pragma unroll
            for (int nt = 0; nt <= NT; nt++) {
                TilePacker e;
                if (nt > 0) mfma_settle(prev);
                if (nt < NT) {
                    f32x16 acc = ini.v;
                    if (nt + 1 < NT) ini.start(prm, pp, nt + 1, hi);
                    if (nt > 0)
                        gemm_reg_act<1>(s, hp, acc, prev, [&](int kb, float r) { e.feed(kb, r); }, [&](int) {});
                    else
                        gemm_reg<NT>(s, hp, acc);
                    gemm_areg<NT>(s, fp, acc, [&](int kb, int g) {
                        if (g == 2 && nt + 1 < NT) ini.step(kb, sx, sy, sz);
                    });
                    if (nt > 0) sl.store(nt - 1, e.p);
                    prev = acc;
                } else {
#pragma unroll
                    for (int kb = 0; kb < 16; kb++) e.feed(kb, softplus100(prev[kb]));
                    sl.store(nt - 1, e.p);
                }
            }
        }
        const float post = i < 2 ? rsqrt2 : 1.0f;
        {
            f32x16 prev;
            RowInit ini, w8;
            const float wsel = i == 2 ? 1.0f : 0.0f;
            ini.v = rp16(prm, pp + 1024, 0, hi);
#pragma unroll
            for (int r = 0; r < 16; r++) w8.v[r] = 0.f;
#pragma unroll
            for (int nt = 0; nt <= NT; nt++) {
                TilePacker e;
                const f32x16 w = w8.v * wsel;
                auto finish = [&](int kb, float v) {
                    const float t = v * post;
                    e.feed(kb, t);
                    out = fmaf(t, w[kb], out);
                };
                if (nt < NT) {
                    f32x16 acc = ini.v;
                    if (nt + 1 < NT) ini.start(prm, pp + 1024, nt + 1, hi);
                    w8.start(prm, P_W8 - W_IB, nt, hi);
                    auto tail = [&](int kb) {
                        if (nt + 1 < NT) ini.step(kb);
                        w8.step(kb);
                    };
                    if (nt > 0)
                        gemm_lds_act<1>(s, sl, acc, prev, [&](int kb, float r) { finish(kb, r); }, tail);
                    else
                        gemm_lds(s, sl, acc, 0, [&](int kb, int g) { if (g == 2) tail(kb); });
                    if (nt > 0) hp[nt - 1] = e.p;
                    prev = acc;
                } else {
                    mfma_settle(prev);
#pragma unroll
                    for (int kb = 0; kb < 16; kb++) finish(kb, softplus100(prev[kb]));
                    hp[nt - 1] = e.p;
                }
            }
        }
    }
    ZS_STAMP(14);
    s.drain();
    out = half_sum(out);
    ZS_STAMP(15);
    return out + prm[P_B8 - W_IB];
}

template <bool GRID>
__global__ __launch_bounds__(WAVES * 64, 1) void sdf_decode_split_kernel(
    const char *__restrict__ programs, size_t program_stride_bytes, int batch,
    const float *__restrict__ points,
    const float *__restrict__ axis,
    int G, long long first_point,
    int m,
    float *__restrict__ out, int apply_sigmoid, f32x4 *__restrict__ workspace,
    int *__restrict__ tile_flags,
    int static_order,
    const float *__restrict__ block0_tables) {
    __shared__ __attribute__((aligned(16))) float lds[LDS_FLOATS];
    float *prm = lds;
    const int lane = threadIdx.x & 63;
    const int wave = __builtin_amdgcn_readfirstlane(threadIdx.x >> 6);
    u32x4 *stage = reinterpret_cast<u32x4 *>(lds + PRM_WINDOW);
    const unsigned stage_addr = __builtin_amdgcn_readfirstlane(
        (unsigned)(uintptr_t)(__attribute__((address_space(3))) float *)(lds + PRM_WINDOW));
    u32x4 *fl = reinterpret_cast<u32x4 *>(lds + PRM_WINDOW + STAGE_FLOATS) + wave * SLAB_U4 + lane;

    const int tiles_per_img = (m + PTS_PER_BLOCK - 1) / PTS_PER_BLOCK;
    const int total = tiles_per_img * batch;
    int *tile_counter = reinterpret_cast<int *>(workspace + (size_t)MAX_WGS * WAVES * ZSLAB_F4) + 256;
    int *tile_slot = tile_counter + 16 + blockIdx.x;
    const int dyn_tiles = total > (int)gridDim.x ? total - (int)gridDim.x : 0;
    for (int tile = blockIdx.x;;) {
      if (tile < total) {
        const int img = tile / tiles_per_img;
        const int t = tile - img * tiles_per_img;
        const char *prog = programs + (size_t)img * program_stride_bytes;

        const int p = t * PTS_PER_BLOCK + wave * PTS_PER_WAVE + (lane & 31);
        const int pc = p < m ? p : m - 1;
        float px, py, pz;
        if (GRID) {
            const long long gp = first_point + pc;
            const long long gg = (long long)G * G;
            const int ix = (int)(gp / gg);
            const int rem = (int)(gp - (long long)ix * gg);
            const int iy = rem / G;
            const int iz = rem - iy * G;
            px = axis[ix];
            py = axis[iy];
            pz = axis[iz];
        } else {
            const float *q = points + ((size_t)img * m + pc) * 3;
            px = q[0];
            py = q[1];
            pz = q[2];
        }
#ifdef ZS_EXP_TIMING
        unsigned long long *dbg = (blockIdx.x == 0 && threadIdx.x == 0 && tile == 0)
            ? reinterpret_cast<unsigned long long *>(workspace + (size_t)MAX_WGS * WAVES * ZSLAB_F4) : nullptr;
#else
        unsigned long long *dbg = nullptr;
#endif
        float guard = 0.f;
        const float *tbl = block0_tables ? block0_tables + (size_t)img * PRM_WINDOW : nullptr;
        float logit = decode_tile(prog, prm, stage, stage_addr, fl, tbl, px, py, pz, wave, lane, guard, dbg);
        if (apply_sigmoid) logit = 1.0f / (1.0f + expf(-logit));
        const unsigned bad = reinterpret_cast<const unsigned *>(prog)[REC_FLOATS + P_FLAG];
        const bool pt_bad = (__builtin_bit_cast(unsigned, px) & 0x7f800000u) == 0x7f800000u ||
                            (__builtin_bit_cast(unsigned, py) & 0x7f800000u) == 0x7f800000u ||
                            (__builtin_bit_cast(unsigned, pz) & 0x7f800000u) == 0x7f800000u;
        if (bad || pt_bad) logit = __builtin_bit_cast(float, 0x7fc00000u);
        if (tile_flags) {
            const bool over = !(__builtin_bit_cast(unsigned, guard) <= __builtin_bit_cast(unsigned, S_GUARD * S_GUARD));
            if (__builtin_amdgcn_ballot_w64(over || bad != 0) != 0 && lane == 0) tile_flags[tile] = 1;
        }
        if (lane < 32 && p < m) out[(size_t)img * m + p] = logit;
      }
        if (static_order) {
            tile += (int)gridDim.x;
            if (tile >= total) break;
            continue;
        }
        if (threadIdx.x == 0) {
            const int d = __hip_atomic_fetch_add(tile_counter, 1, __ATOMIC_RELAXED, __HIP_MEMORY_SCOPE_AGENT);
            if (d == dyn_tiles + (int)gridDim.x - 1)
                __hip_atomic_store(tile_counter, 0, __ATOMIC_RELAXED, __HIP_MEMORY_SCOPE_AGENT);
            __hip_atomic_store(tile_slot, d, __ATOMIC_RELAXED, __HIP_MEMORY_SCOPE_AGENT);
        }
        __syncthreads();
        const int d = __builtin_amdgcn_readfirstlane(__hip_atomic_load(tile_slot, __ATOMIC_RELAXED, __HIP_MEMORY_SCOPE_AGENT));
        if ((unsigned)d >= (unsigned)dyn_tiles) break;
        tile = (int)gridDim.x + d;
    }
}

DEV bool out_of_range(const f32x4 &v) {
    const unsigned lim = 0x477fe000u;
    return (__builtin_bit_cast(unsigned, v.x) & 0x7fffffffu) > lim || (__builtin_bit_cast(unsigned, v.y) & 0x7fffffffu) > lim ||
           (__builtin_bit_cast(unsigned, v.z) & 0x7fffffffu) > lim || (__builtin_bit_cast(unsigned, v.w) & 0x7fffffffu) > lim;
}

__host__ __device__ inline int split_source_kblock(int kb) {
    constexpr int KB_BLOCK = G_BLOCK / 2, KB_ATT = HEADS * G_HEAD / 2;
    static_assert(KB_BLOCK - KB_ATT == HT * 32, "an MLP section is 32 K-blocks per hidden tile");
    constexpr int KB_IMPL0 = BLOCKS * KB_BLOCK, KB_L = NT * NT * 2;
    if (kb >= KB_IMPL0 + G_IMPL / 2) return kb;
    if (kb >= KB_IMPL0) {
        const int p = kb - KB_IMPL0;
        if (p < KB_L) return kb;
        if (p < 2 * KB_L) return KB_IMPL0 + 4 * KB_L + (p - KB_L);
        const int q = p - 2 * KB_L, pair = q / (3 * KB_L), r = q - pair * 3 * KB_L;
        if (r >= 2 * KB_L) return KB_IMPL0 + (5 + 2 * pair + 1) * KB_L + (r - 2 * KB_L);
        const int nt = r / (4 * NT), w = r - nt * 4 * NT;
        return w < 2 * NT ? KB_IMPL0 + (5 + 2 * pair) * KB_L + nt * 2 * NT + w
                          : KB_IMPL0 + (1 + pair) * KB_L + nt * 2 * NT + (w - 2 * NT);
    }
    const int blk = kb / KB_BLOCK, p = kb - blk * KB_BLOCK - KB_ATT;
    if (p < 16) return kb;
    const int q = p - 16, it = q >> 5, r = q & 31;
    int src;
    if (it < HT - 1)
        src = r < 16 ? (it + 1) * 32 + r : it * 32 + r;
    else
        src = it * 32 + 16 + r;
    return blk * KB_BLOCK + KB_ATT + src;
}

__global__ __launch_bounds__(256) void split_program_kernel(const float *__restrict__ src,
                                                            size_t src_stride_floats,
                                                            u32x4 *__restrict__ dst,
                                                            size_t dst_stride_u4) {
    const int img = blockIdx.y;
    const float *s = src + (size_t)img * src_stride_floats;
    u32x4 *d = dst + (size_t)img * dst_stride_u4;
    const int e = blockIdx.x * 256 + threadIdx.x;
    constexpr int REC_KB = REC_FLOATS / (KB_U4 * 4);
    if (e < REC_KB * 64) {
        const int kb = e >> 6, lane = e & 63;
        const f32x4 *g = reinterpret_cast<const f32x4 *>(s) + (size_t)split_source_kblock(kb) * 128;
        const f32x4 a = g[lane], b = g[64 + lane];
        if (out_of_range(a) || out_of_range(b)) atomicOr(reinterpret_cast<unsigned *>(d) + REC_FLOATS + P_FLAG, 1u);
        unsigned h[4], l[4];
        split2(a.x, a.y, h[0], l[0]);
        split2(a.z, a.w, h[1], l[1]);
        split2(b.x, b.y, h[2], l[2]);
        split2(b.z, b.w, h[3], l[3]);
        const u32x4 hi = {h[0], h[1], h[2], h[3]}, lo = {l[0], l[1], l[2], l[3]};
        d[(size_t)kb * KB_U4 + lane] = hi;
        d[(size_t)kb * KB_U4 + 64 + lane] = lo;
    } else {
        const int i = e - REC_KB * 64;
        if (i < PARAM_FLOATS / 4 && i != P_FLAG / 4 && (i < P_KMAX / 4 || i >= (P_KMAX + BLOCKS * HEADS) / 4)) {
            const f32x4 v = reinterpret_cast<const f32x4 *>(s + REC_FLOATS)[i];
            if (i < (P_USED + 3) / 4 && out_of_range(v))
                atomicOr(reinterpret_cast<unsigned *>(d) + REC_FLOATS + P_FLAG, 1u);
            d[REC_FLOATS / 4 + i] = __builtin_bit_cast(u32x4, v);
        }
    }
}

__global__ __launch_bounds__(256) void k_bound_kernel(const float *__restrict__ src, size_t src_stride_floats,
                                                      u32x4 *__restrict__ dst, size_t dst_stride_u4) {
    __shared__ float red[256];
    const int img = blockIdx.y, bh = blockIdx.x, blk = bh / HEADS, hd = bh - blk * HEADS;
    const float *kv = src + (size_t)img * src_stride_floats +
                      (size_t)(blk * G_BLOCK + hd * G_HEAD + G_QKV_HEAD) * GROUP_FLOATS;
    float sq = 0.f;
    const int t = threadIdx.x;
    if (t < LT * 32) {
        const int lt = t >> 5;
#pragma unroll
        for (int half = 0; half < 2; half++)
#pragma unroll
            for (int g = 0; g < 4; g++) {
                const f32x4 v = reinterpret_cast<const f32x4 *>(kv + (lt * 8 + g) * GROUP_FLOATS)[(t & 31) + 32 * half];
                sq = fmaf(v.x, v.x, fmaf(v.y, v.y, fmaf(v.z, v.z, fmaf(v.w, v.w, sq))));
            }
    }
    red[t] = sq;
    __syncthreads();
    for (int o = 128; o > 0; o >>= 1) {
        if (t < o) red[t] = fmaxf(red[t], red[t + o]);
        __syncthreads();
    }
    if (t == 0)
        reinterpret_cast<float *>(dst + (size_t)img * dst_stride_u4)[REC_FLOATS + P_KMAX + bh] = sqrtf(red[0]);
}

constexpr int B0_THREADS = 256;
__global__ __launch_bounds__(B0_THREADS) void block0_window_kernel(const char *__restrict__ programs,
                                                                   size_t program_stride_bytes, float *__restrict__ tables) {
    __shared__ double red[B0_THREADS][5];
    __shared__ double msum[64][4];
    const int tile = blockIdx.x, img = blockIdx.y, t = threadIdx.x, wave = t >> 6, lane = t & 63, hl = lane >> 5;
    const char *prog = programs + (size_t)img * program_stride_bytes;
    const float *par = reinterpret_cast<const float *>(prog) + REC_FLOATS;
    float *out = tables + (size_t)img * PRM_WINDOW;
    if (t < 64) {
#pragma unroll
        for (int d = 0; d < 4; d++) {
            double a = 0.0;
#pragma unroll
            for (int f = 0; f < 4; f++) a += (double)par[P_PP + (4 * t + f) * 4 + d];
            msum[t][d] = a;
        }
    }
    __syncthreads();
    double m[4] = {0.0, 0.0, 0.0, 0.0};
    for (int i = 0; i < 64; i++)
#pragma unroll
        for (int d = 0; d < 4; d++) m[d] += msum[i][d];
#pragma unroll
    for (int d = 0; d < 4; d++) m[d] *= 1.0 / C;
    const int head = tile / 3, part = tile - head * 3;
    const u32x4 *kb0 = reinterpret_cast<const u32x4 *>(prog) + (size_t)(head * (G_HEAD / 2) + part * 2 * NT) * KB_U4;
    double acc[5] = {0.0, 0.0, 0.0, 0.0, 0.0};
#pragma unroll
    for (int k = 0; k < 4; k++) {
        const int kb = 4 * wave + k;
        const u32x4 h4 = kb0[kb * KB_U4 + lane], l4 = kb0[kb * KB_U4 + 64 + lane];
        const int f0 = (kb >> 1) * 32 + hl * 16 + (kb & 1) * 8;
#pragma unroll
        for (int e = 0; e < 8; e++) {
            const unsigned hw = h4[e >> 1] >> (16 * (e & 1)), lw = l4[e >> 1] >> (16 * (e & 1));
            const double w = (double)(float)__builtin_bit_cast(_Float16, (unsigned short)hw) +
                             (double)(float)__builtin_bit_cast(_Float16, (unsigned short)lw);
            const double wg = w * (double)par[P_BLK0 + PB_LN1G + f0 + e];
#pragma unroll
            for (int d = 0; d < 4; d++) acc[d] += wg * ((double)par[P_PP + (f0 + e) * 4 + d] - m[d]);
            acc[4] += w * (double)par[P_BLK0 + PB_LN1B + f0 + e];
        }
    }
#pragma unroll
    for (int d = 0; d < 5; d++) red[t][d] = acc[d];
    __syncthreads();
    if (t < 32) {
        const int hh = (t >> 2) & 1, r = (t & 3) + 4 * (t >> 3), o = tile * 32 + hh * 16 + r;
        double sum[5] = {0.0, 0.0, 0.0, 0.0, 0.0};
        for (int w = 0; w < B0_THREADS / 64; w++)
#pragma unroll
            for (int d = 0; d < 5; d++) sum[d] += red[w * 64 + t][d] + red[w * 64 + 32 + t][d];
#pragma unroll
        for (int d = 0; d < 4; d++) out[B0_T + o * 4 + d] = (float)sum[d];
        out[B0_C + o] = (float)(sum[4] + (double)par[P_BLK0 + PB_BQKV + o]);
    }
    if (tile < C / 32 && t < 32) out[B0_BPROJ + tile * 32 + t] = par[P_BLK0 + PB_BPROJ + tile * 32 + t];
}

const float *launch_block0_tables(const void *split_programs, size_t program_stride_bytes, int batch, void *workspace,
                                  hipStream_t st) {
    const char *e = getenv("ZS_SPLIT_BLOCK0_GEMM");
    if (e && atoi(e) != 0) return nullptr;
    if ((size_t)batch * PRM_WINDOW * sizeof(float) > (size_t)MAX_WGS * WAVES * ZSLAB_F4 * sizeof(f32x4)) return nullptr;
    float *tables = static_cast<float *>(workspace);
    hipLaunchKernelGGL(block0_window_kernel, dim3(HEADS * 3, batch), dim3(B0_THREADS), 0, st,
                       static_cast<const char *>(split_programs), program_stride_bytes, tables);
    return tables;
}

int decode_grid_size(int batch, int m) {
    const long long tiles = (long long)batch * ((m + PTS_PER_BLOCK - 1) / PTS_PER_BLOCK);
    return (int)(tiles < MAX_WGS ? tiles : MAX_WGS);
}

bool check_programs(const char *what, const void *programs, size_t stride) {
    if (!programs) {
        zs::set_err("%s: null pointer", what);
        return false;
    }
    if (stride % 16 != 0 || stride < zs_sdf_program_bytes()) {
        zs::set_err("%s: bad program stride %zu", what, stride);
        return false;
    }
    return true;
}

}

extern "C" int zs_sdf_split_programs(const void *programs, size_t program_stride_bytes,
                                     void *split_programs, size_t split_stride_bytes, int batch,
                                     void *stream) {
    if (batch < 0 || batch > 65535) {
        zs::set_err("zs_sdf_split_programs: bad batch %d", batch);
        return 0;
    }
    if (batch == 0) return 1;
    if (!check_programs("zs_sdf_split_programs", programs, program_stride_bytes) ||
        !check_programs("zs_sdf_split_programs", split_programs, split_stride_bytes))
        return 0;
    const int elems = (REC_FLOATS / (KB_U4 * 4)) * 64 + PARAM_FLOATS / 4;
    hipStream_t st = static_cast<hipStream_t>(stream);
    if (hipMemset2DAsync(static_cast<char *>(split_programs) + (size_t)(REC_FLOATS + P_FLAG) * 4, split_stride_bytes,
                         0, 16, batch, st) != hipSuccess) {
        zs::set_err("zs_sdf_split_programs: hipMemset2DAsync failed");
        return 0;
    }
    hipLaunchKernelGGL(split_program_kernel, dim3((elems + 255) / 256, batch), dim3(256), 0, st,
                       static_cast<const float *>(programs), program_stride_bytes / sizeof(float),
                       static_cast<u32x4 *>(split_programs), split_stride_bytes / sizeof(u32x4));
    hipLaunchKernelGGL(k_bound_kernel, dim3(BLOCKS * HEADS, batch), dim3(256), 0, st,
                       static_cast<const float *>(programs), program_stride_bytes / sizeof(float),
                       static_cast<u32x4 *>(split_programs), split_stride_bytes / sizeof(u32x4));
    return zs::check_launch("zs_sdf_split_programs") ? 1 : 0;
}

extern "C" int zs_sdf_block0_tables(const void *split_programs, size_t program_stride_bytes, int batch, float *tables,
                                    void *stream) {
    if (batch < 0 || batch > 65535) {
        zs::set_err("zs_sdf_block0_tables: bad batch %d", batch);
        return 0;
    }
    if (batch == 0) return 1;
    if (!tables) {
        zs::set_err("zs_sdf_block0_tables: null pointer");
        return 0;
    }
    if (!check_programs("zs_sdf_block0_tables", split_programs, program_stride_bytes)) return 0;
    hipLaunchKernelGGL(block0_window_kernel, dim3(HEADS * 3, batch), dim3(B0_THREADS), 0, static_cast<hipStream_t>(stream),
                       static_cast<const char *>(split_programs), program_stride_bytes, tables);
    return zs::check_launch("zs_sdf_block0_tables") ? 1 : 0;
}

static int launch_counter_reset(void *workspace, hipStream_t st) {
    const char *e = getenv("ZS_SPLIT_STATIC_TILES");
    if (e && atoi(e) != 0) return 1;
    int *tile_counter = reinterpret_cast<int *>(static_cast<f32x4 *>(workspace) + (size_t)MAX_WGS * WAVES * ZSLAB_F4) + 256;
    (void)hipMemsetAsync(tile_counter, 0, sizeof(int), st);
    return 0;
}

extern "C" int zs_sdf_query_points_split(const void *split_programs, size_t program_stride_bytes,
                                         int batch, const float *points, int m, float *logits,
                                         int *tile_flags, void *workspace, void *stream) {
    if (batch < 0 || m < 0) {
        zs::set_err("zs_sdf_query_points_split: negative size (batch=%d m=%d)", batch, m);
        return 0;
    }
    if (batch == 0 || m == 0) return 1;
    if (!points || !logits || !workspace) {
        zs::set_err("zs_sdf_query_points_split: null pointer");
        return 0;
    }
    if (!check_programs("zs_sdf_query_points_split", split_programs, program_stride_bytes)) return 0;
    if ((long long)batch * ((m + PTS_PER_BLOCK - 1) / PTS_PER_BLOCK) > 0x7fffffffLL) {
        zs::set_err("zs_sdf_query_points_split: too many tiles");
        return 0;
    }
    const int static_order = launch_counter_reset(workspace, static_cast<hipStream_t>(stream));
    const float *b0_tables = launch_block0_tables(split_programs, program_stride_bytes, batch, workspace, static_cast<hipStream_t>(stream));
    hipLaunchKernelGGL((sdf_decode_split_kernel<false>), dim3(decode_grid_size(batch, m)),
                       dim3(WAVES * 64), 0, static_cast<hipStream_t>(stream),
                       static_cast<const char *>(split_programs), program_stride_bytes, batch, points,
                       nullptr, 0, 0LL, m, logits, 0, static_cast<f32x4 *>(workspace), tile_flags, static_order, b0_tables);
    return zs::check_launch("zs_sdf_query_points_split") ? 1 : 0;
}

extern "C" int zs_sdf_query_grid_range_split(const void *split_programs, size_t program_stride_bytes,
                                             int batch, const float *axis, int G, long long point_begin,
                                             long long point_end, int apply_sigmoid, float *out,
                                             int *tile_flags, void *workspace, void *stream) {
    const long long P = (long long)G * G * G;
    if (batch < 0 || G <= 0 || point_begin < 0 || point_end > P || point_begin > point_end) {
        zs::set_err("zs_sdf_query_grid_range_split: bad range (batch=%d G=%d points=[%lld,%lld))", batch, G,
                    point_begin, point_end);
        return 0;
    }
    const long long mm = point_end - point_begin;
    if (batch == 0 || mm == 0) return 1;
    if (!axis || !out || !workspace) {
        zs::set_err("zs_sdf_query_grid_range_split: null pointer");
        return 0;
    }
    if (mm > 0x7fffffffLL - PTS_PER_BLOCK) {
        zs::set_err("zs_sdf_query_grid_range_split: %lld points per launch exceed 2^31; split the range", mm);
        return 0;
    }
    if (!check_programs("zs_sdf_query_grid_range_split", split_programs, program_stride_bytes)) return 0;
    const int m = (int)mm;
    const int static_order = launch_counter_reset(workspace, static_cast<hipStream_t>(stream));
    const float *b0_tables = launch_block0_tables(split_programs, program_stride_bytes, batch, workspace, static_cast<hipStream_t>(stream));
    hipLaunchKernelGGL((sdf_decode_split_kernel<true>), dim3(decode_grid_size(batch, m)),
                       dim3(WAVES * 64), 0, static_cast<hipStream_t>(stream),
                       static_cast<const char *>(split_programs), program_stride_bytes, batch, nullptr,
                       axis, G, point_begin, m, out, apply_sigmoid, static_cast<f32x4 *>(workspace), tile_flags, static_order, b0_tables);
    return zs::check_launch("zs_sdf_query_grid_range_split") ? 1 : 0;
}

extern "C" int zs_sdf_query_grid_split(const void *split_programs, size_t program_stride_bytes,
                                       int batch, const float *axis, int G, int slice_begin,
                                       int slice_end, int apply_sigmoid, float *out, int *tile_flags,
                                       void *workspace, void *stream) {
    if (batch < 0 || G <= 0 || slice_begin < 0 || slice_end > G || slice_begin > slice_end) {
        zs::set_err("zs_sdf_query_grid_split: bad range (batch=%d G=%d slices=[%d,%d))", batch, G,
                    slice_begin, slice_end);
        return 0;
    }
    const long long mm = (long long)(slice_end - slice_begin) * G * G;
    if (batch == 0 || mm == 0) return 1;
    if (!axis || !out || !workspace) {
        zs::set_err("zs_sdf_query_grid_split: null pointer");
        return 0;
    }
    if (mm > 0x7fffffffLL - PTS_PER_BLOCK) {
        zs::set_err("zs_sdf_query_grid_split: %lld points per launch exceed 2^31; split the slab", mm);
        return 0;
    }
    if (!check_programs("zs_sdf_query_grid_split", split_programs, program_stride_bytes)) return 0;
    const int m = (int)mm;
    const int static_order = launch_counter_reset(workspace, static_cast<hipStream_t>(stream));
    const float *b0_tables = launch_block0_tables(split_programs, program_stride_bytes, batch, workspace, static_cast<hipStream_t>(stream));
    hipLaunchKernelGGL((sdf_decode_split_kernel<true>), dim3(decode_grid_size(batch, m)),
                       dim3(WAVES * 64), 0, static_cast<hipStream_t>(stream),
                       static_cast<const char *>(split_programs), program_stride_bytes, batch, nullptr,
                       axis, G, (long long)slice_begin * G * G, m, out, apply_sigmoid,
                       static_cast<f32x4 *>(workspace), tile_flags, static_order, b0_tables);
    return zs::check_launch("zs_sdf_query_grid_split") ? 1 : 0;
}
```

### zeroshape_amd/program.py

```python
import numpy as np

C = 256
NT = C // 32
HEADS = 8
HD = 32
L = 197
LT = 7
HID = 1024
HT = HID // 32
BLOCKS = 2
MLP_LAYERS = 9
SKIP_IN = (2, 4, 6)
GROUP_FLOATS = 256
RING = 8

LANE = np.arange(64)
LANE_I = LANE & 31
LANE_HI = LANE >> 5


def row(r, hi):
    return (r & 3) + 8 * (r >> 2) + 4 * hi


ROW_TABLE = np.array([[row(r, hi) for r in range(16)] for hi in range(2)])


def _records_linear(W, nt, kt):
    rows = 32 * nt + LANE_I
    cols = 32 * kt + ROW_TABLE[LANE_HI][:, :].T
    return W[rows[None, :], cols]


def _interleave(recs):
    n = recs.shape[0]
    assert n % 4 == 0
    return recs.reshape(n // 4, 4, 64).transpose(0, 2, 1).reshape(-1)


def records_for_linear(W, n_out_tiles=None, k_tiles=None):
    W = np.asarray(W, np.float32)
    n_out_tiles = W.shape[0] // 32 if n_out_tiles is None else n_out_tiles
    k_tiles = W.shape[1] // 32 if k_tiles is None else k_tiles
    out = [_records_linear(W, nt, kt) for nt in range(n_out_tiles) for kt in range(k_tiles)]
    return np.concatenate(out, axis=0)


def kv_records(K_h, V_h):
    Kp = np.zeros((LT * 32, HD), np.float32)
    Vp = np.zeros((LT * 32, HD), np.float32)
    Kp[:L], Vp[:L] = K_h, V_h
    out = []
    for lt in range(LT):
        krec = Kp[(32 * lt + LANE_I)[None, :], ROW_TABLE[LANE_HI].T]
        vrec = Vp[32 * lt + ROW_TABLE[LANE_HI].T, LANE_I[None, :]]
        out += [krec, vrec]
    return np.concatenate(out, axis=0)


G_QKV_HEAD = 3 * NT * 4
G_KV_HEAD = LT * 8
G_PROJ_HEAD = NT * 4
G_HEAD = G_QKV_HEAD + G_KV_HEAD + G_PROJ_HEAD
G_MLP_TILE = NT * 4 + NT * 4
G_BLOCK = HEADS * G_HEAD + HT * G_MLP_TILE
G_IMPL_PLAIN = NT * NT * 4
G_IMPL_SKIP = 2 * G_IMPL_PLAIN
G_IMPL = G_IMPL_PLAIN * 5 + G_IMPL_SKIP * 3
G_TOTAL = BLOCKS * G_BLOCK + G_IMPL
REC_FLOATS = (G_TOTAL + RING) * GROUP_FLOATS
PARAM_FLOATS = 13824
PROGRAM_FLOATS = REC_FLOATS + PARAM_FLOATS
PROGRAM_BYTES = PROGRAM_FLOATS * 4


def kv_group_offset(blk, head):
    return blk * G_BLOCK + head * G_HEAD + G_QKV_HEAD


def pack_records(sd, kv=None):
    out = []
    for blk in range(BLOCKS):
        p = "blocks_attn.%d." % blk
        Wqkv = np.asarray(sd[p + "attn.qkv.weight"], np.float32)
        Wproj = np.asarray(sd[p + "attn.proj.weight"], np.float32)
        W1 = np.asarray(sd[p + "mlp.fc1.weight"], np.float32)
        W2 = np.asarray(sd[p + "mlp.fc2.weight"], np.float32)
        for h in range(HEADS):
            for part in range(3):
                Wt = Wqkv[part * C + h * HD: part * C + (h + 1) * HD]
                out.append(records_for_linear(Wt))
            if kv is not None:
                out.append(kv_records(*kv[(blk, h)]))
            else:
                out.append(np.zeros((G_KV_HEAD * 4, 64), np.float32))
            out.append(records_for_linear(Wproj[:, h * HD:(h + 1) * HD]))
        for ht in range(HT):
            out.append(records_for_linear(W1[ht * 32:(ht + 1) * 32]))
            out.append(records_for_linear(W2[:, ht * 32:(ht + 1) * 32]))
    Wl = [np.asarray(sd["impl_mlp.layers.%d.weight" % l], np.float32) for l in range(MLP_LAYERS)]
    out.append(records_for_linear(Wl[0][:, 3:]))
    for l in SKIP_IN:
        out.append(records_for_linear(Wl[l][:, C + 3:]))
    for l in range(1, MLP_LAYERS - 1):
        if l in SKIP_IN:
            out.append(records_for_linear(Wl[l][:, :C]))
        else:
            out.append(records_for_linear(Wl[l]))
    recs = np.concatenate(out, axis=0)
    assert recs.shape == (G_TOTAL * 4, 64), recs.shape
    flat = _interleave(recs)
    out = np.concatenate([flat, np.zeros(RING * GROUP_FLOATS, np.float32)])
    assert out.size == REC_FLOATS
    return out


def rowparam(v):
    v = np.asarray(v, np.float32)
    T = v.shape[0] // 32
    idx = (32 * np.arange(T))[:, None, None] + ROW_TABLE[None, :, :]
    return v[idx].reshape(-1)


def rowparam4(cols):
    stacked = np.stack([rowparam(c).reshape(-1) for c in cols], axis=-1)
    return stacked.reshape(-1)


class ParamLayout(object):

    def __init__(self):
        o = 0

        def take(n):
            nonlocal o
            s = o
            o += n
            return s
        self.PP = take(C * 4)
        self.blk = []
        for _ in range(BLOCKS):
            d = {}
            d["ln1_g"] = take(C)
            d["ln1_b"] = take(C)
            d["bproj"] = take(C)
            d["bqkv"] = take(HEADS * 3 * 32)
            d["ln2_g"] = take(C)
            d["ln2_b"] = take(C)
            d["b2"] = take(C)
            d["b1"] = take(HID)
            self.blk.append(d)
        self.lnf_g = take(C)
        self.lnf_b = take(C)
        self.impl = []
        for l in range(MLP_LAYERS - 1):
            if l == 0 or l in SKIP_IN:
                self.impl.append(take(C * 4))
            else:
                self.impl.append(take(C))
        self.w8 = take(C)
        self.b8 = take(16)
        self.total = o


PARAMS = ParamLayout()
assert PARAMS.total <= PARAM_FLOATS
P_FLAG = 13600
P_KMAX = 13616
assert PARAMS.total <= P_FLAG and P_FLAG + 4 <= P_KMAX and P_KMAX + BLOCKS * HEADS <= PARAM_FLOATS
BLOCK_PARAM_FLOATS = 3 * C + HEADS * 96 + 3 * C + HID


def pack_params(sd):
    g = lambda k: np.asarray(sd[k], np.float32)
    out = np.zeros(PARAM_FLOATS, np.float32)

    def put(off, arr):
        out[off:off + arr.size] = arr
    Wp = g("point_proj.proj.weight")
    put(PARAMS.PP, rowparam4([Wp[:, 0], Wp[:, 1], Wp[:, 2], g("point_proj.proj.bias")]))
    for blk in range(BLOCKS):
        p, d = "blocks_attn.%d." % blk, PARAMS.blk[blk]
        put(d["ln1_g"], rowparam(g(p + "norm1.weight")))
        put(d["ln1_b"], rowparam(g(p + "norm1.bias")))
        put(d["bproj"], rowparam(g(p + "attn.proj.bias")))
        bq = g(p + "attn.qkv.bias")
        parts = []
        for h in range(HEADS):
            for part in range(3):
                parts.append(rowparam(bq[part * C + h * HD: part * C + (h + 1) * HD]))
        put(d["bqkv"], np.concatenate(parts))
        put(d["ln2_g"], rowparam(g(p + "norm2.weight")))
        put(d["ln2_b"], rowparam(g(p + "norm2.bias")))
        put(d["b2"], rowparam(g(p + "mlp.fc2.bias")))
        put(d["b1"], rowparam(g(p + "mlp.fc1.bias")))
    put(PARAMS.lnf_g, rowparam(g("norm.weight")))
    put(PARAMS.lnf_b, rowparam(g("norm.bias")))
    for l in range(MLP_LAYERS - 1):
        W, b = g("impl_mlp.layers.%d.weight" % l), g("impl_mlp.layers.%d.bias" % l)
        if l == 0:
            put(PARAMS.impl[l], rowparam4([W[:, 0], W[:, 1], W[:, 2], b]))
        elif l in SKIP_IN:
            put(PARAMS.impl[l], rowparam4([W[:, C], W[:, C + 1], W[:, C + 2], b]))
        else:
            put(PARAMS.impl[l], rowparam(b))
    put(PARAMS.w8, rowparam(g("impl_mlp.layers.8.weight")[0]))
    out[PARAMS.b8] = g("impl_mlp.layers.8.bias")[0]
    return out


def pack_program(sd, kv=None):
    out = np.concatenate([pack_records(sd, kv), pack_params(sd)])
    assert out.size == PROGRAM_FLOATS
    return out


class LatentLayout(object):
    def __init__(self, latent_dim=C):
        o = 0

        def take(n):
            nonlocal o
            s = o
            o += n
            return s
        self.latent_dim = latent_dim
        self.Wlp = take(latent_dim * C)
        self.blp = take(C)
        self.pos = take(L * C)
        self.ln1g0 = take(C)
        self.ln1b0 = take(C)
        self.Wqkv0 = take(C * 3 * C)
        self.bqkv0 = take(3 * C)
        self.Wproj0 = take(C * C)
        self.bproj0 = take(C)
        self.ln2g0 = take(C)
        self.ln2b0 = take(C)
        self.W1 = take(C * HID)
        self.b1 = take(HID)
        self.W2 = take(HID * C)
        self.b2 = take(C)
        self.ln1g1 = take(C)
        self.ln1b1 = take(C)
        self.Wkv1 = take(C * 2 * C)
        self.bkv1 = take(2 * C)
        self.total = o


LATENT = LatentLayout()


def pack_latent_params(sd):
    g = lambda k: np.asarray(sd[k], np.float32)
    assert g("latent_proj.weight").shape == (C, LATENT.latent_dim)
    out = np.zeros(LATENT.total, np.float32)

    def put(off, arr):
        arr = np.ascontiguousarray(arr, np.float32).reshape(-1)
        out[off:off + arr.size] = arr
    put(LATENT.Wlp, g("latent_proj.weight").T)
    put(LATENT.blp, g("latent_proj.bias"))
    put(LATENT.pos, g("pos_embed").reshape(L, C))
    b0, b1 = "blocks_attn.0.", "blocks_attn.1."
    put(LATENT.ln1g0, g(b0 + "norm1.weight"))
    put(LATENT.ln1b0, g(b0 + "norm1.bias"))
    put(LATENT.Wqkv0, g(b0 + "attn.qkv.weight").T)
    put(LATENT.bqkv0, g(b0 + "attn.qkv.bias"))
    put(LATENT.Wproj0, g(b0 + "attn.proj.weight").T)
    put(LATENT.bproj0, g(b0 + "attn.proj.bias"))
    put(LATENT.ln2g0, g(b0 + "norm2.weight"))
    put(LATENT.ln2b0, g(b0 + "norm2.bias"))
    put(LATENT.W1, g(b0 + "mlp.fc1.weight").T)
    put(LATENT.b1, g(b0 + "mlp.fc1.bias"))
    put(LATENT.W2, g(b0 + "mlp.fc2.weight").T)
    put(LATENT.b2, g(b0 + "mlp.fc2.bias"))
    put(LATENT.ln1g1, g(b1 + "norm1.weight"))
    put(LATENT.ln1b1, g(b1 + "norm1.bias"))
    put(LATENT.Wkv1, g(b1 + "attn.qkv.weight")[C:].T)
    put(LATENT.bkv1, g(b1 + "attn.qkv.bias")[C:])
    return out


LPAD = 200
SCRATCH_FLOATS = LPAD * (3 * C + 3 * C + C + HID + 2 * C)


KB_TOTAL = G_TOTAL // 2
KB_WORDS = 512


def split_source_kblocks(n=None):
    n = REC_FLOATS // GROUP_FLOATS // 2 if n is None else n
    src = np.arange(n)
    kb_block, kb_att = G_BLOCK // 2, HEADS * G_HEAD // 2
    order = list(range(16))
    for t in range(HT - 1):
        order += [(t + 1) * 32 + r for r in range(16)] + [t * 32 + 16 + r for r in range(16)]
    order += [(HT - 1) * 32 + 16 + r for r in range(16)]
    assert sorted(order) == list(range(HT * 32))
    for blk in range(BLOCKS):
        base = blk * kb_block + kb_att
        src[base:base + HT * 32] = base + np.array(order)
    b0, kl = BLOCKS * kb_block, NT * NT * 2
    impl = list(range(kl)) + [4 * kl + i for i in range(kl)]
    for pair in range(3):
        for nt in range(NT):
            impl += [(5 + 2 * pair) * kl + nt * 2 * NT + w for w in range(2 * NT)]
            impl += [(1 + pair) * kl + nt * 2 * NT + w for w in range(2 * NT)]
        impl += [(6 + 2 * pair) * kl + i for i in range(kl)]
    assert sorted(impl) == list(range(G_IMPL // 2))
    src[b0:b0 + G_IMPL // 2] = b0 + np.array(impl)
    return src


def f16_round(x):
    x = np.ascontiguousarray(x, np.float32)
    with np.errstate(over="ignore"):
        h = x.astype(np.float16)
    return h.view(np.uint16), h.astype(np.float32)


def f16_rtz(x):
    x = np.ascontiguousarray(x, np.float32)
    with np.errstate(over="ignore"):
        h = x.astype(np.float16)
    away = np.abs(h.astype(np.float32)) > np.abs(x)
    h = np.where(away, np.nextafter(h, np.float16(0)), h).astype(np.float16)
    return h.view(np.uint16), h.astype(np.float32)


def split_program(prog):
    prog = np.ascontiguousarray(prog, np.float32)
    rec = prog[:REC_FLOATS].reshape(-1, 2, 64, 4)
    rec = rec[split_source_kblocks(rec.shape[0])]
    vals = rec.transpose(0, 2, 1, 3).reshape(-1, 64, 8)
    hi16, hif = f16_round(vals)
    with np.errstate(invalid="ignore"):
        lo16, _ = f16_round(vals - hif)
    out = np.stack([hi16, lo16], axis=1)
    words = np.ascontiguousarray(out).reshape(-1).view(np.uint32)
    params = prog[REC_FLOATS:].copy()
    params[P_KMAX:P_KMAX + BLOCKS * HEADS] = latent_k_bounds(prog).reshape(-1)
    bad = not (np.all(np.isfinite(prog)) and float(np.abs(prog).max()) <= F16_MAX)
    params[P_FLAG:P_FLAG + 1].view(np.uint32)[0] = 1 if bad else 0
    return np.concatenate([words, params.view(np.uint32)])


S_GUARD = 64.0
W_MAX = 16.0
F16_MAX = 65504.0


def split_envelope(sd):
    vals = [np.asarray(v, np.float32) for k, v in sd.items() if k != "pos_embed"]
    wmax = max(float(np.max(np.abs(v))) if np.all(np.isfinite(v)) else float("inf") for v in vals)
    return wmax <= W_MAX, dict(max_abs_weight=wmax)


def latent_k_bounds(prog):
    prog = np.ascontiguousarray(prog, np.float32)
    out = np.zeros((BLOCKS, HEADS), np.float32)
    for blk in range(BLOCKS):
        for h in range(HEADS):
            o = kv_group_offset(blk, h) * GROUP_FLOATS
            g = prog[o:o + G_KV_HEAD * GROUP_FLOATS].reshape(LT, 8, 64, 4)[:, :4]
            rec = g.transpose(0, 1, 3, 2).reshape(LT, 16, 64)
            sq = (rec.astype(np.float64) ** 2).sum(1)
            row = sq[:, :32] + sq[:, 32:]
            out[blk, h] = np.sqrt(row.max())
    return out


B0_WINDOW_FLOATS = 4096
B0_BPROJ, B0_C, B0_T = 0, C, C + HEADS * 96
KB_HEAD = G_HEAD // 2
KB_QKV_HEAD = G_QKV_HEAD // 2


def _kblock_values(words, kb):
    h = np.ascontiguousarray(words[kb * KB_WORDS:(kb + 1) * KB_WORDS]).view(np.float16).reshape(2, 64, 8)
    return h[0].astype(np.float64) + h[1].astype(np.float64)


def block0_qkv_weights(split_prog):
    W = np.zeros((3 * C, C), np.float64)
    for h in range(HEADS):
        for part in range(3):
            for kt in range(NT):
                for j in range(2):
                    v = _kblock_values(split_prog, h * KB_HEAD + part * 2 * NT + kt * 2 + j)
                    rows = part * C + h * HD + LANE_I
                    cols = 32 * kt + ROW_TABLE[LANE_HI][:, 8 * j:8 * j + 8]
                    W[rows[:, None], cols] = v
    return W


def _from_rowparam(v):
    v = np.asarray(v)
    T = v.shape[0] // 32
    idx = ((32 * np.arange(T))[:, None, None] + ROW_TABLE[None, :, :]).reshape(-1)
    out = np.empty_like(v)
    out[idx] = v
    return out


def block0_window(split_prog):
    words = np.ascontiguousarray(split_prog).view(np.uint32)
    params = words[REC_FLOATS:].view(np.float32).astype(np.float64)
    d = PARAMS.blk[0]
    A = np.stack([_from_rowparam(params[PARAMS.PP + i:PARAMS.PP + 4 * C:4]) for i in range(4)], axis=1)
    g = _from_rowparam(params[d["ln1_g"]:d["ln1_g"] + C])
    b = _from_rowparam(params[d["ln1_b"]:d["ln1_b"] + C])
    W = block0_qkv_weights(words)
    T = W @ (g[:, None] * (A - A.mean(axis=0, keepdims=True)))
    c = W @ b
    out = np.zeros(B0_WINDOW_FLOATS, np.float64)
    out[B0_BPROJ:B0_BPROJ + C] = params[d["bproj"]:d["bproj"] + C]
    for h in range(HEADS):
        for part in range(3):
            tile = 3 * h + part
            rows = slice(part * C + h * HD, part * C + (h + 1) * HD)
            out[B0_C + tile * 32:B0_C + (tile + 1) * 32] = \
                _rowparam64(c[rows]) + params[d["bqkv"] + tile * 32:d["bqkv"] + (tile + 1) * 32]
            out[B0_T + tile * 128:B0_T + (tile + 1) * 128] = \
                np.stack([_rowparam64(T[rows, i]) for i in range(4)], axis=-1).reshape(-1)
    return out.astype(np.float32)


def _rowparam64(v):
    v = np.asarray(v, np.float64)
    T = v.shape[0] // 32
    idx = (32 * np.arange(T))[:, None, None] + ROW_TABLE[None, :, :]
    return v[idx].reshape(-1)


def split_consumed_kblocks():
    keep = [kb for kb in range(KB_TOTAL) if not (kb < HEADS * KB_HEAD and kb % KB_HEAD < KB_QKV_HEAD)]
    return np.array(keep)
```

Measured before the change: 75.71 million.

## Precompute block-0 attention logit tables to replace QK gemm with one MFMA

Adds a per-image precompute kernel that folds the block-0 LayerNorm/QKV affine map into the key matrix, giving a small G table (5 columns per key) stored as hi/lo f16 pairs. In the decode kernel, block-0 attention scores become a single 32x32x16 MFMA of this table against a per-point packed [x,y,z,rstd,1] operand, instead of a two-step K-block gemm. The G tiles are DMA'd into the staging ring in place of K blocks, with a per-image usable flag falling back to the old path on f16 overflow. This adds an extra launch and tricky stream bookkeeping, and the f16 hi/lo split carries some accuracy risk.

```diff
diff --git a/include/zeroshape_hip.h b/include/zeroshape_hip.h
--- a/include/zeroshape_hip.h
+++ b/include/zeroshape_hip.h
@@ -8,7 +8,7 @@
 extern "C" {
 #endif
 
-#define ZS_ABI_VERSION 41
+#define ZS_ABI_VERSION 42
 
 int zs_abi_version(void);
 
@@ -73,6 +73,9 @@
                             void *stream);
 
 int zs_sdf_block0_tables(const void *split_programs, size_t program_stride_bytes, int batch, float *tables, void *stream);
+
+int zs_sdf_block0_logit_tables(const void *split_programs, size_t program_stride_bytes, int batch, void *logit_tables,
+                               int *usable, void *stream);
 
 int zs_sdf_query_grid_range(const void *programs, size_t program_stride_bytes, int batch,
                             const float *axis, int G, long long point_begin, long long point_end,
diff --git a/zeroshape_amd/_lib.py b/zeroshape_amd/_lib.py
--- a/zeroshape_amd/_lib.py
+++ b/zeroshape_amd/_lib.py
@@ -52,6 +52,7 @@
                                 _c_void_p, _c_void_p]),
     "zs_sdf_split_programs": (_c_int, [_c_void_p, _c_size_t, _c_void_p, _c_size_t, _c_int, _c_void_p]),
     "zs_sdf_block0_tables": (_c_int, [_c_void_p, _c_size_t, _c_int, _c_void_p, _c_void_p]),
+    "zs_sdf_block0_logit_tables": (_c_int, [_c_void_p, _c_size_t, _c_int, _c_void_p, _c_void_p, _c_void_p]),
     "zs_sdf_query_points_split": (_c_int, [_c_void_p, _c_size_t, _c_int, _c_void_p, _c_int,
                                            _c_void_p, _c_void_p, _c_void_p, _c_void_p]),
     "zs_sdf_query_grid_split": (_c_int, [_c_void_p, _c_size_t, _c_int, _c_void_p, _c_int, _c_int,
@@ -211,7 +212,7 @@
     "zs_readout_concat_bwd": (_c_int, [_c_void_p, _c_void_p, _c_int, _c_int, _c_int, _c_void_p]),
 }
 
-ABI_VERSION = 41
+ABI_VERSION = 42
 _lib = None
 
 
diff --git a/zeroshape_amd/csrc/sdf_decoder_split.hip b/zeroshape_amd/csrc/sdf_decoder_split.hip
--- a/zeroshape_amd/csrc/sdf_decoder_split.hip
+++ b/zeroshape_amd/csrc/sdf_decoder_split.hip
@@ -95,28 +95,48 @@
                  : "memory");
 }
 
+DEV void glds_gtile(const char *gtile, unsigned lane16, unsigned lds_dst) {
+#ifdef ZS_EXP_NO_DMA
+    if (gtile != nullptr) return;
+#endif
+    asm volatile("s_mov_b32 m0, %2\n\ts_nop 0\n\tglobal_load_lds_dwordx4 %0, %1" ZS_DMA_MOD
+                 :
+                 : "v"(lane16), "s"(gtile), "s"(lds_dst)
+                 : "memory");
+}
+
 struct AStream {
     const u32x4 *buf[NBUF];
     unsigned dst[NBUF];
     u32x4 hi, lo;
     const char *gsrc;
-
-    DEV void init(const char *prog, u32x4 *stage, unsigned stage_addr, int wave, int lane, int first_byte = 0) {
+    unsigned lane16;
+
+    DEV void init(const char *prog, u32x4 *stage, unsigned stage_addr, int wave, int lane, int first_byte = 0,
+                  bool lg = false, const char *g0 = nullptr, const char *g1 = nullptr) {
         const char *g = prog + first_byte + wave * (KPW * KB_U4 * 16) + lane * 16;
+        lane16 = lane * 16;
         asm volatile("s_waitcnt vmcnt(0) lgkmcnt(0)\n\ts_barrier" ::: "memory");
 #pragma unroll
         for (int i = 0; i < NBUF; i++) {
             buf[i] = stage + i * (CK * KB_U4) + lane;
             dst[i] = stage_addr + i * CHUNK_BYTES + wave * (KPW * KB_U4 * 16);
-            glds_kblocks(g + i * CHUNK_BYTES, dst[i]);
+            const char *gi = i == 0 ? g0 : g1;
+            if (gi)
+                glds_gtile(gi, lane16, dst[i]);
+            else
+                glds_kblocks(g + i * CHUNK_BYTES, dst[i]);
         }
         gsrc = g + NBUF * CHUNK_BYTES;
-        asm volatile("s_waitcnt vmcnt(4)\n\ts_barrier" ::: "memory");
+        if (lg)
+            asm volatile("s_waitcnt vmcnt(0)\n\ts_barrier" ::: "memory");
+        else
+            asm volatile("s_waitcnt vmcnt(4)\n\ts_barrier" ::: "memory");
         hi = buf[0][0];
         lo = buf[0][64];
     }
     template <int EXTRA_VM = 0>
-    DEV void step(int pos, u32x4 &ahi, u32x4 &alo) {
+    DEV void step(int pos, u32x4 &ahi, u32x4 &alo, const char *gt = nullptr) {
         ahi = hi;
         alo = lo;
         if (pos == CK - 1) {
@@ -125,7 +145,10 @@
                 asm volatile("s_waitcnt vmcnt(4) lgkmcnt(0)\n\ts_barrier" ::: "memory");
             else
                 asm volatile("s_waitcnt vmcnt(0) lgkmcnt(0)\n\ts_barrier" ::: "memory");
-            glds_kblocks(gsrc, dst[0]);
+            if (gt)
+                glds_gtile(gt, lane16, dst[0]);
+            else
+                glds_kblocks(gsrc, dst[0]);
             gsrc += CHUNK_BYTES;
             const u32x4 *t = buf[0];
             const unsigned u = dst[0];
@@ -141,6 +164,11 @@
             lo = buf[0][(pos + 1) * KB_U4 + 64];
 #endif
         }
+    }
+    DEV void step_g(int pos, u32x4 &g) {
+        g = hi;
+        hi = buf[0][(pos + 2) * KB_U4];
+        lo = buf[0][(pos + 2) * KB_U4 + 64];
     }
     DEV void skip(int bytes) { gsrc += bytes; }
     DEV void drain() { asm volatile("s_waitcnt vmcnt(0) lgkmcnt(0)" ::: "memory"); }
@@ -356,11 +384,11 @@
     ZS_FENCE;
 }
 template <bool YACC = false, typename SIDE = NoSide>
-DEV void gemm_one(AStream &s, const PT &X, f32x16 &acc, int pos0, int kb0 = 0, SIDE side = SIDE()) {
+DEV void gemm_one(AStream &s, const PT &X, f32x16 &acc, int pos0, int kb0 = 0, SIDE side = SIDE(), const char *gt = nullptr) {
 #pragma unroll
     for (int j = 0; j < 2; j++) {
         u32x4 ahi, alo;
-        s.step((pos0 + j) & (CK - 1), ahi, alo);
+        s.step((pos0 + j) & (CK - 1), ahi, alo, gt);
         pin(ahi, alo);
         if (YACC)
             mfma3_cacc(acc, ahi, alo, X.v[2 * j], X.v[2 * j + 1], kb0 + j, side);
@@ -480,6 +508,8 @@
     }
     return v;
 }
+constexpr int G_TILE_BYTES = 64 * 16;
+constexpr int G_IMG_BYTES = HEADS * LT * G_TILE_BYTES;
 DEV f32x16 xyz_affine(const float *prm, int off, int tile, int hi, float x, float y, float z) {
     const f32x4 *q = reinterpret_cast<const f32x4 *>(prm + off + tile * 128 + hi * 64);
     f32x16 v;
@@ -563,9 +593,16 @@
 
 template <bool MASK>
 DEV void attn_tile(AStream &s, const PT &q, f32x16 &o, float &m_run, float &z_run, float c, int hi,
-                   int pos0) {
+                   int pos0, bool lg = false, const char *gt = nullptr) {
     f32x16 S = zero16();
-    gemm_one(s, q, S, pos0);
+    if (lg) {
+        u32x4 g;
+        s.step_g(pos0, g);
+        asm volatile("" : "+v"(g) : : "memory");
+        S = __builtin_amdgcn_mfma_f32_32x32x16_f16(zs::s16::as_h(g), zs::s16::as_h(q.v[0]), S, 0, 0, 0);
+    } else {
+        gemm_one(s, q, S, pos0);
+    }
     float mt = -INFINITY;
 #pragma unroll
     for (int r = 0; r < 16; r++) {
@@ -594,7 +631,7 @@
         zs_ += p;
     }
     z_run += zs_;
-    gemm_one(s, pack_tile(S), o, pos0 + 2);
+    gemm_one(s, pack_tile(S), o, pos0 + 2, 0, NoSide(), gt);
 }
 
 #ifdef ZS_EXP_TIMING
@@ -603,14 +640,19 @@
 #define ZS_STAMP(i) do { } while (0)
 #endif
 DEV float decode_tile(const char *prog, float *prm, u32x4 *stage, unsigned stage_addr, u32x4 *slab,
-                      const float *tbl, float px, float py, float pz, int wave, int lane, float &guard,
+                      const float *tbl, const char *gtab, float px, float py, float pz, int wave, int lane, float &guard,
                       unsigned long long *dbg) {
     const int hi = lane >> 5;
     const float *prog_params = reinterpret_cast<const float *>(prog) + REC_FLOATS;
     constexpr int QKV_BYTES = 3 * NT * 2 / CK * CHUNK_BYTES;
     static_assert(3 * NT * 2 % CK == 0, "AStream::skip passes whole chunks");
+    const bool lg = gtab != nullptr;
+    auto gop = [&](bool on, int w0, int w2) -> const char * {
+        const int idx = wave == 0 ? w0 : wave == 2 ? w2 : -1;
+        return on && idx >= 0 ? gtab + idx * G_TILE_BYTES : nullptr;
+    };
     AStream s;
-    s.init(prog, stage, stage_addr, wave, lane, tbl ? QKV_BYTES : 0);
+    s.init(prog, stage, stage_addr, wave, lane, tbl ? QKV_BYTES : 0, lg, gop(lg, 0, 1), gop(lg, 2, 3));
     Slab sl;
     sl.fl = slab;
     ZS_STAMP(0);
@@ -627,6 +669,7 @@
 #pragma unroll 1
     for (int blk = 0; blk < BLOCKS; blk++) {
         const bool tab = blk == 0 && tbl != nullptr;
+        const bool lgt = blk == 0 && lg;
         float rstd0 = 0.f, xr = 0.f, yr = 0.f, zr = 0.f;
         if (tab) {
             load_params(prm, tbl, 0, PRM_WINDOW);
@@ -672,16 +715,31 @@
                 const float km = prog_params[P_KMAX + blk * HEADS + hd] * scale;
                 guard = fmaxf(guard, half_sum(qq) * (km * km));
             }
-            const PT qp = pack_tile(q);
+            PT qp;
+            if (lgt) {
+                const unsigned h01 = zs::s16::pk_f16(xr, yr), h23 = zs::s16::pk_f16(zr, rstd0);
+                auto f16v = [](unsigned w) { return (float)__builtin_bit_cast(_Float16, (unsigned short)w); };
+                const unsigned l01 = zs::s16::pk_f16(fmaf(px, rstd0, -f16v(h01)), fmaf(py, rstd0, -f16v(h01 >> 16)));
+                const unsigned l23 = zs::s16::pk_f16(fmaf(pz, rstd0, -f16v(h23)), rstd0 - f16v(h23 >> 16));
+                const unsigned one = 0x3c00u;
+                const u32x4 ub = hi ? u32x4{h01, h23, one | (l23 & 0xffff0000u), (l23 >> 16) | (l01 << 16)}
+                                    : u32x4{h01, h23, one | (l01 << 16), (l01 >> 16) | (l23 << 16)};
+#pragma unroll
+                for (int i = 0; i < 4; i++) qp.v[i] = ub;
+            } else {
+                qp = pack_tile(q);
+            }
 
             float m_run = -INFINITY, z_run = 0.f;
             f32x16 o = zero16();
 #pragma unroll 1
             for (int l2 = 0; l2 < (LT - 1) / 2; l2++) {
-                attn_tile<false>(s, qp, o, m_run, z_run, c, hi, P);
-                attn_tile<false>(s, qp, o, m_run, z_run, c, hi, (P + 4) & (CK - 1));
+                const char *gt = P == 0 ? gop(lgt, l2 < 2 ? hd * LT + 2 * l2 + 4 : -1, l2 == 0 ? hd * LT + 5 : -1)
+                                        : gop(lgt && l2 < 2, hd * LT + 2 * l2 + 3, hd * LT + 2 * l2 + 4);
+                attn_tile<false>(s, qp, o, m_run, z_run, c, hi, P, lgt, P == 4 ? gt : nullptr);
+                attn_tile<false>(s, qp, o, m_run, z_run, c, hi, (P + 4) & (CK - 1), lgt, P == 0 ? gt : nullptr);
             }
-            attn_tile<true>(s, qp, o, m_run, z_run, c, hi, P);
+            attn_tile<true>(s, qp, o, m_run, z_run, c, hi, P, lgt);
             {
                 const float m_new = fmaxf(m_run, s_self);
                 const float alpha = __builtin_amdgcn_exp2f(m_run - m_new);
@@ -698,7 +756,12 @@
 #pragma unroll
             for (int nt = 0; nt < NT; nt++) {
                 if (P == 0 && nt == 2 && bump && wave < 2) s.skip(QKV_BYTES);
-                gemm_one(s, op, y[nt], (P + 4 + 2 * nt) & (CK - 1));
+                const char *gt = nullptr;
+                if (P == 0 && nt == 1) gt = gop(lgt, -1, (hd + 1) * LT);
+                if (P == 0 && nt == 5) gt = gop(lgt, (hd + 1) * LT + 1, (hd + 1) * LT + 2);
+                if (P == 4 && nt == 3) gt = gop(lgt && bump, (hd + 1) * LT, (hd + 1) * LT + 1);
+                if (P == 4 && nt == 7) gt = gop(lgt && bump, (hd + 1) * LT + 2, (hd + 1) * LT + 3);
+                gemm_one(s, op, y[nt], (P + 4 + 2 * nt) & (CK - 1), 0, NoSide(), gt);
             }
         };
         static_assert((LT - 1) % 2 == 0 && (3 * NT * 2 + LT * 4 + NT * 2) % CK == 4, "head = 11.5 chunks");
@@ -913,7 +976,8 @@
     float *__restrict__ out, int apply_sigmoid, f32x4 *__restrict__ workspace,
     int *__restrict__ tile_flags,
     int static_order,
-    const float *__restrict__ block0_tables) {
+    const float *__restrict__ block0_tables,
+    const char *__restrict__ block0_logits) {
     __shared__ __attribute__((aligned(16))) float lds[LDS_FLOATS];
     float *prm = lds;
     const int lane = threadIdx.x & 63;
@@ -961,7 +1025,11 @@
 #endif
         float guard = 0.f;
         const float *tbl = block0_tables ? block0_tables + (size_t)img * PRM_WINDOW : nullptr;
-        float logit = decode_tile(prog, prm, stage, stage_addr, fl, tbl, px, py, pz, wave, lane, guard, dbg);
+        const char *gtab = nullptr;
+        if (tbl && block0_logits &&
+            reinterpret_cast<const int *>(block0_logits + (size_t)batch * G_IMG_BYTES)[img] != 0)
+            gtab = block0_logits + (size_t)img * G_IMG_BYTES;
+        float logit = decode_tile(prog, prm, stage, stage_addr, fl, tbl, gtab, px, py, pz, wave, lane, guard, dbg);
         if (apply_sigmoid) logit = 1.0f / (1.0f + expf(-logit));
         const unsigned bad = reinterpret_cast<const unsigned *>(prog)[REC_FLOATS + P_FLAG];
         const bool pt_bad = (__builtin_bit_cast(unsigned, px) & 0x7f800000u) == 0x7f800000u ||
@@ -1086,14 +1154,9 @@
 }
 
 constexpr int B0_THREADS = 256;
-__global__ __launch_bounds__(B0_THREADS) void block0_window_kernel(const char *__restrict__ programs,
-                                                                   size_t program_stride_bytes, float *__restrict__ tables) {
-    __shared__ double red[B0_THREADS][5];
-    __shared__ double msum[64][4];
-    const int tile = blockIdx.x, img = blockIdx.y, t = threadIdx.x, wave = t >> 6, lane = t & 63, hl = lane >> 5;
-    const char *prog = programs + (size_t)img * program_stride_bytes;
+DEV void block0_tile_sums(const char *prog, int tile, double (*red)[5], double (*msum)[4], double *sum) {
+    const int t = threadIdx.x, wave = t >> 6, lane = t & 63, hl = lane >> 5;
     const float *par = reinterpret_cast<const float *>(prog) + REC_FLOATS;
-    float *out = tables + (size_t)img * PRM_WINDOW;
     if (t < 64) {
 #pragma unroll
         for (int d = 0; d < 4; d++) {
@@ -1132,12 +1195,25 @@
 #pragma unroll
     for (int d = 0; d < 5; d++) red[t][d] = acc[d];
     __syncthreads();
+#pragma unroll
+    for (int d = 0; d < 5; d++) sum[d] = 0.0;
+    if (t < 32)
+        for (int w = 0; w < B0_THREADS / 64; w++)
+#pragma unroll
+            for (int d = 0; d < 5; d++) sum[d] += red[w * 64 + t][d] + red[w * 64 + 32 + t][d];
+}
+__global__ __launch_bounds__(B0_THREADS) void block0_window_kernel(const char *__restrict__ programs,
+                                                                   size_t program_stride_bytes, float *__restrict__ tables) {
+    __shared__ double red[B0_THREADS][5];
+    __shared__ double msum[64][4];
+    const int tile = blockIdx.x, img = blockIdx.y, t = threadIdx.x;
+    const char *prog = programs + (size_t)img * program_stride_bytes;
+    const float *par = reinterpret_cast<const float *>(prog) + REC_FLOATS;
+    float *out = tables + (size_t)img * PRM_WINDOW;
+    double sum[5];
+    block0_tile_sums(prog, tile, red, msum, sum);
     if (t < 32) {
         const int hh = (t >> 2) & 1, r = (t & 3) + 4 * (t >> 3), o = tile * 32 + hh * 16 + r;
-        double sum[5] = {0.0, 0.0, 0.0, 0.0, 0.0};
-        for (int w = 0; w < B0_THREADS / 64; w++)
-#pragma unroll
-            for (int d = 0; d < 5; d++) sum[d] += red[w * 64 + t][d] + red[w * 64 + 32 + t][d];
 #pragma unroll
         for (int d = 0; d < 4; d++) out[B0_T + o * 4 + d] = (float)sum[d];
         out[B0_C + o] = (float)(sum[4] + (double)par[P_BLK0 + PB_BQKV + o]);
@@ -1145,15 +1221,95 @@
     if (tile < C / 32 && t < 32) out[B0_BPROJ + tile * 32 + t] = par[P_BLK0 + PB_BPROJ + tile * 32 + t];
 }
 
-const float *launch_block0_tables(const void *split_programs, size_t program_stride_bytes, int batch, void *workspace,
+__global__ __launch_bounds__(B0_THREADS) void block0_logit_kernel(const char *__restrict__ programs, size_t program_stride_bytes,
+                                                                  char *__restrict__ logits, int *__restrict__ usable) {
+    __shared__ double red[B0_THREADS][5];
+    __shared__ double msum[64][4];
+    __shared__ double tq[32][5];
+    __shared__ double half1[32][5];
+    __shared__ float gf[32][5];
+    const int lt = blockIdx.x % LT, head = blockIdx.x / LT, img = blockIdx.y, t = threadIdx.x, lane = t & 63, hl = lane >> 5;
+    const char *prog = programs + (size_t)img * program_stride_bytes;
+    const float *par = reinterpret_cast<const float *>(prog) + REC_FLOATS;
+    double sum[5];
+    block0_tile_sums(prog, 3 * head, red, msum, sum);
+    if (t < 32) {
+        const int hh = (t >> 2) & 1, r = (t & 3) + 4 * (t >> 3);
+#pragma unroll
+        for (int d = 0; d < 4; d++) tq[t][d] = sum[d];
+        tq[t][4] = sum[4] + (double)par[P_BLK0 + PB_BQKV + 3 * head * 32 + hh * 16 + r];
+    }
+    __syncthreads();
+    double acc[5] = {0.0, 0.0, 0.0, 0.0, 0.0};
+    if (t < 64) {
+        const u32x4 *kb0 = reinterpret_cast<const u32x4 *>(prog) +
+                           (size_t)(head * (G_HEAD / 2) + G_QKV_HEAD / 2 + lt * 4) * KB_U4;
+#pragma unroll
+        for (int j = 0; j < 2; j++) {
+            const u32x4 h4 = kb0[j * KB_U4 + lane], l4 = kb0[j * KB_U4 + 64 + lane];
+#pragma unroll
+            for (int e = 0; e < 8; e++) {
+                const unsigned hw = h4[e >> 1] >> (16 * (e & 1)), lw = l4[e >> 1] >> (16 * (e & 1));
+                const double k = (double)(float)__builtin_bit_cast(_Float16, (unsigned short)hw) +
+                                 (double)(float)__builtin_bit_cast(_Float16, (unsigned short)lw);
+                const int r = 8 * j + e, dim = (r & 3) + 8 * (r >> 2) + 4 * hl;
+#pragma unroll
+                for (int d = 0; d < 5; d++) acc[d] += k * tq[dim][d];
+            }
+        }
+        if (hl == 1)
+#pragma unroll
+            for (int d = 0; d < 5; d++) half1[lane & 31][d] = acc[d];
+    }
+    __syncthreads();
+    if (t < 32)
+#pragma unroll
+        for (int d = 0; d < 5; d++) gf[t][d] = 32 * lt + t < L ? (float)(acc[d] + half1[t][d]) : 0.f;
+    __syncthreads();
+    if (t >= 64) return;
+    float g[5];
+    bool bad = false;
+#pragma unroll
+    for (int d = 0; d < 5; d++) {
+        g[d] = gf[lane & 31][d];
+        bad = bad || (__builtin_bit_cast(unsigned, g[d]) & 0x7fffffffu) > 0x477fe000u;
+    }
+    unsigned gh[3], gl[3];
+    split2(g[0], g[1], gh[0], gl[0]);
+    split2(g[2], g[3], gh[1], gl[1]);
+    split2(g[4], 0.f, gh[2], gl[2]);
+    const u32x4 a = hl == 0 ? u32x4{gh[0], gh[1], (gh[2] & 0xffffu) | (gh[0] << 16), (gh[0] >> 16) | (gh[1] << 16)}
+                            : u32x4{gl[0], gl[1], (gl[2] & 0xffffu) | (gh[1] & 0xffff0000u), (gl[1] >> 16) | (gl[0] << 16)};
+    reinterpret_cast<u32x4 *>(logits + (size_t)img * G_IMG_BYTES + (size_t)(head * LT + lt) * G_TILE_BYTES)[lane] = a;
+    if (bad) atomicAnd(usable + img, 0);
+}
+
+struct Block0Tables {
+    const float *windows;
+    const char *logits;
+};
+Block0Tables launch_block0_tables(const void *split_programs, size_t program_stride_bytes, int batch, void *workspace,
                                   hipStream_t st) {
+    Block0Tables r = {nullptr, nullptr};
     const char *e = getenv("ZS_SPLIT_BLOCK0_GEMM");
-    if (e && atoi(e) != 0) return nullptr;
-    if ((size_t)batch * PRM_WINDOW * sizeof(float) > (size_t)MAX_WGS * WAVES * ZSLAB_F4 * sizeof(f32x4)) return nullptr;
+    if (e && atoi(e) != 0) return r;
+    const size_t region = (size_t)MAX_WGS * WAVES * ZSLAB_F4 * sizeof(f32x4);
+    const size_t win_bytes = (size_t)batch * PRM_WINDOW * sizeof(float);
+    if (win_bytes > region) return r;
     float *tables = static_cast<float *>(workspace);
     hipLaunchKernelGGL(block0_window_kernel, dim3(HEADS * 3, batch), dim3(B0_THREADS), 0, st,
                        static_cast<const char *>(split_programs), program_stride_bytes, tables);
-    return tables;
+    r.windows = tables;
+    e = getenv("ZS_SPLIT_BLOCK0_SGEMM");
+    if (e && atoi(e) != 0) return r;
+    if (win_bytes + (size_t)batch * (G_IMG_BYTES + sizeof(int)) > region) return r;
+    char *logits = static_cast<char *>(workspace) + win_bytes;
+    int *usable = reinterpret_cast<int *>(logits + (size_t)batch * G_IMG_BYTES);
+    if (hipMemsetD32Async(reinterpret_cast<hipDeviceptr_t>(usable), 1, batch, st) != hipSuccess) return r;
+    hipLaunchKernelGGL(block0_logit_kernel, dim3(HEADS * LT, batch), dim3(B0_THREADS), 0, st,
+                       static_cast<const char *>(split_programs), program_stride_bytes, logits, usable);
+    r.logits = logits;
+    return r;
 }
 
 int decode_grid_size(int batch, int m) {
@@ -1219,6 +1375,29 @@
     return zs::check_launch("zs_sdf_block0_tables") ? 1 : 0;
 }
 
+extern "C" int zs_sdf_block0_logit_tables(const void *split_programs, size_t program_stride_bytes, int batch,
+                                          void *logit_tables, int *usable, void *stream) {
+    if (batch < 0 || batch > 65535) {
+        zs::set_err("zs_sdf_block0_logit_tables: bad batch %d", batch);
+        return 0;
+    }
+    if (batch == 0) return 1;
+    if (!logit_tables || !usable) {
+        zs::set_err("zs_sdf_block0_logit_tables: null pointer");
+        return 0;
+    }
+    if (!check_programs("zs_sdf_block0_logit_tables", split_programs, program_stride_bytes)) return 0;
+    hipStream_t st = static_cast<hipStream_t>(stream);
+    if (hipMemsetD32Async(reinterpret_cast<hipDeviceptr_t>(usable), 1, batch, st) != hipSuccess) {
+        zs::set_err("zs_sdf_block0_logit_tables: hipMemsetD32Async failed");
+        return 0;
+    }
+    hipLaunchKernelGGL(block0_logit_kernel, dim3(HEADS * LT, batch), dim3(B0_THREADS), 0, st,
+                       static_cast<const char *>(split_programs), program_stride_bytes,
+                       static_cast<char *>(logit_tables), usable);
+    return zs::check_launch("zs_sdf_block0_logit_tables") ? 1 : 0;
+}
+
 static int launch_counter_reset(void *workspace, hipStream_t st) {
     const char *e = getenv("ZS_SPLIT_STATIC_TILES");
     if (e && atoi(e) != 0) return 1;
@@ -1245,11 +1424,11 @@
         return 0;
     }
     const int static_order = launch_counter_reset(workspace, static_cast<hipStream_t>(stream));
-    const float *b0_tables = launch_block0_tables(split_programs, program_stride_bytes, batch, workspace, static_cast<hipStream_t>(stream));
+    const Block0Tables b0 = launch_block0_tables(split_programs, program_stride_bytes, batch, workspace, static_cast<hipStream_t>(stream));
     hipLaunchKernelGGL((sdf_decode_split_kernel<false>), dim3(decode_grid_size(batch, m)),
                        dim3(WAVES * 64), 0, static_cast<hipStream_t>(stream),
                        static_cast<const char *>(split_programs), program_stride_bytes, batch, points,
-                       nullptr, 0, 0LL, m, logits, 0, static_cast<f32x4 *>(workspace), tile_flags, static_order, b0_tables);
+                       nullptr, 0, 0LL, m, logits, 0, static_cast<f32x4 *>(workspace), tile_flags, static_order, b0.windows, b0.logits);
     return zs::check_launch("zs_sdf_query_points_split") ? 1 : 0;
 }
 
@@ -1276,11 +1455,11 @@
     if (!check_programs("zs_sdf_query_grid_range_split", split_programs, program_stride_bytes)) return 0;
     const int m = (int)mm;
     const int static_order = launch_counter_reset(workspace, static_cast<hipStream_t>(stream));
-    const float *b0_tables = launch_block0_tables(split_programs, program_stride_bytes, batch, workspace, static_cast<hipStream_t>(stream));
+    const Block0Tables b0 = launch_block0_tables(split_programs, program_stride_bytes, batch, workspace, static_cast<hipStream_t>(stream));
     hipLaunchKernelGGL((sdf_decode_split_kernel<true>), dim3(decode_grid_size(batch, m)),
                        dim3(WAVES * 64), 0, static_cast<hipStream_t>(stream),
                        static_cast<const char *>(split_programs), program_stride_bytes, batch, nullptr,
-                       axis, G, point_begin, m, out, apply_sigmoid, static_cast<f32x4 *>(workspace), tile_flags, static_order, b0_tables);
+                       axis, G, point_begin, m, out, apply_sigmoid, static_cast<f32x4 *>(workspace), tile_flags, static_order, b0.windows, b0.logits);
     return zs::check_launch("zs_sdf_query_grid_range_split") ? 1 : 0;
 }
 
@@ -1306,11 +1485,11 @@
     if (!check_programs("zs_sdf_query_grid_split", split_programs, program_stride_bytes)) return 0;
     const int m = (int)mm;
     const int static_order = launch_counter_reset(workspace, static_cast<hipStream_t>(stream));
-    const float *b0_tables = launch_block0_tables(split_programs, program_stride_bytes, batch, workspace, static_cast<hipStream_t>(stream));
+    const Block0Tables b0 = launch_block0_tables(split_programs, program_stride_bytes, batch, workspace, static_cast<hipStream_t>(stream));
     hipLaunchKernelGGL((sdf_decode_split_kernel<true>), dim3(decode_grid_size(batch, m)),
                        dim3(WAVES * 64), 0, static_cast<hipStream_t>(stream),
                        static_cast<const char *>(split_programs), program_stride_bytes, batch, nullptr,
                        axis, G, (long long)slice_begin * G * G, m, out, apply_sigmoid,
-                       static_cast<f32x4 *>(workspace), tile_flags, static_order, b0_tables);
+                       static_cast<f32x4 *>(workspace), tile_flags, static_order, b0.windows, b0.logits);
     return zs::check_launch("zs_sdf_query_grid_split") ? 1 : 0;
 }
diff --git a/zeroshape_amd/program.py b/zeroshape_amd/program.py
--- a/zeroshape_amd/program.py
+++ b/zeroshape_amd/program.py
@@ -404,8 +404,7 @@
     return out
 
 
-def block0_window(split_prog):
-    words = np.ascontiguousarray(split_prog).view(np.uint32)
+def _block0_tc(words):
     params = words[REC_FLOATS:].view(np.float32).astype(np.float64)
     d = PARAMS.blk[0]
     A = np.stack([_from_rowparam(params[PARAMS.PP + i:PARAMS.PP + 4 * C:4]) for i in range(4)], axis=1)
@@ -414,6 +413,13 @@
     W = block0_qkv_weights(words)
     T = W @ (g[:, None] * (A - A.mean(axis=0, keepdims=True)))
     c = W @ b
+    return T, c, params
+
+
+def block0_window(split_prog):
+    words = np.ascontiguousarray(split_prog).view(np.uint32)
+    T, c, params = _block0_tc(words)
+    d = PARAMS.blk[0]
     out = np.zeros(B0_WINDOW_FLOATS, np.float64)
     out[B0_BPROJ:B0_BPROJ + C] = params[d["bproj"]:d["bproj"] + C]
     for h in range(HEADS):
@@ -437,3 +443,60 @@
 def split_consumed_kblocks():
     keep = [kb for kb in range(KB_TOTAL) if not (kb < HEADS * KB_HEAD and kb % KB_HEAD < KB_QKV_HEAD)]
     return np.array(keep)
+
+
+KB_S_HEAD = LT * 4
+G_SLOT_COL = np.array([0, 1, 2, 3, 4, 0, 1, 2, 0, 1, 2, 3, 4, 3, 3, 0])
+G_SLOT_HALF = np.array([0, 0, 0, 0, 0, 0, 0, 0, 1, 1, 1, 1, 1, 0, 1, 1])
+G_SLOT_UHALF = np.array([0, 0, 0, 0, 0, 1, 1, 1, 0, 0, 0, 0, 0, 1, 1, 1])
+G_TILE_WORDS = 256
+G_IMG_WORDS = HEADS * LT * G_TILE_WORDS
+
+
+def block0_logit_g(split_prog):
+    words = np.ascontiguousarray(split_prog).view(np.uint32)
+    T, c, params = _block0_tc(words)
+    bq = PARAMS.blk[0]["bqkv"]
+    G = np.zeros((HEADS, LT * 32, 5), np.float64)
+    with np.errstate(invalid="ignore", over="ignore"):
+        for h in range(HEADS):
+            rows = slice(h * HD, (h + 1) * HD)
+            cq = _rowparam64(c[rows]) + params[bq + 3 * h * 32:bq + (3 * h + 1) * 32]
+            tc = np.concatenate([np.stack([_rowparam64(T[rows, i]) for i in range(4)], axis=-1), cq[:, None]],
+                                axis=-1).reshape(2, 16, 5)
+            for lt in range(LT):
+                for j in range(2):
+                    k = _kblock_values(words, h * KB_HEAD + KB_QKV_HEAD + lt * 4 + j)
+                    for hl in range(2):
+                        G[h, 32 * lt:32 * lt + 32] += k[32 * hl:32 * hl + 32] @ tc[hl, 8 * j:8 * j + 8]
+        G[:, L:] = 0.0
+        return G.astype(np.float32)
+
+
+def block0_logit_table(split_prog):
+    G = block0_logit_g(split_prog)
+    usable = bool(np.all(np.isfinite(G)) and float(np.abs(G).max()) <= F16_MAX)
+    hi16, hif = f16_round(G)
+    with np.errstate(invalid="ignore"):
+        lo16, _ = f16_round(G - hif)
+    halves = np.stack([hi16, lo16], axis=0)
+    ops = np.zeros((HEADS, LT * 32, 16), np.uint16)
+    for s in range(16):
+        ops[:, :, s] = halves[G_SLOT_HALF[s], :, :, G_SLOT_COL[s]]
+    ops = ops.reshape(HEADS, LT, 32, 2, 8).transpose(0, 1, 3, 2, 4)
+    return np.ascontiguousarray(ops).reshape(HEADS, LT, 64, 8).view(np.uint32), usable
+
+
+def block0_logit_decode(ops):
+    v = np.ascontiguousarray(ops).view(np.float16).reshape(HEADS, LT, 2, 32, 8)
+    slots = v.transpose(0, 1, 3, 2, 4).reshape(HEADS, LT * 32, 16).astype(np.float32)
+    G = np.zeros((HEADS, LT * 32, 5), np.float64)
+    for col in range(5):
+        hi = int(np.flatnonzero((G_SLOT_COL == col) & (G_SLOT_HALF == 0))[0])
+        lo = int(np.flatnonzero((G_SLOT_COL == col) & (G_SLOT_HALF == 1))[0])
+        G[:, :, col] = slots[:, :, hi].astype(np.float64) + slots[:, :, lo].astype(np.float64)
+    return G, slots
+
+
+def split_block0_logit_slots():
+    return np.array([h * KB_HEAD + KB_QKV_HEAD + lt * 4 + j for h in range(HEADS) for lt in range(LT) for j in range(2)])
```

New measurement: 75.96 million (median of 6 runs). No clear change (+0.3%).
